# google-deepmind/mujoco_warp

Hardware: NVIDIA H100
Metric: env-steps/sec (whole box) on humanoid.xml at nworld=8192 per GPU (higher is better)
Workload: dtype f32

## Files before the change

### mujoco_warp_b200/_src/io.py

```python

from __future__ import annotations

import weakref

import numpy as np
import torch

from . import _lib
from . import constants as C
from . import mjcf
from . import types

_FLOAT_FIELDS = [
  "qpos0", "qpos_spring", "body_pos", "body_quat", "body_ipos", "body_iquat", "body_mass", "body_subtreemass",
  "body_inertia", "body_invweight0", "body_gravcomp", "jnt_pos", "jnt_axis", "jnt_stiffness", "jnt_range", "jnt_margin", "jnt_solref",
  "jnt_solimp", "jnt_actfrcrange", "dof_armature", "dof_damping", "dof_invweight0", "dof_frictionloss", "dof_solref",
  "dof_solimp", "geom_size", "geom_aabb", "geom_rbound", "geom_pos", "geom_quat", "geom_friction", "geom_margin",
  "geom_gap", "geom_solmix", "geom_solref", "geom_solimp", "actuator_gear", "actuator_gainprm", "actuator_biasprm",
  "actuator_ctrlrange", "actuator_forcerange", "cam_pos", "cam_quat", "cam_poscom0", "cam_pos0", "cam_mat0",
  "light_pos", "light_dir", "light_poscom0", "light_pos0", "light_dir0", "site_pos", "site_quat",
]
_INT_FIELDS = [
  "body_parentid", "body_rootid", "body_weldid", "body_mocapid", "body_jntnum", "body_jntadr", "body_dofnum", "body_dofadr",
  "jnt_type", "jnt_qposadr", "jnt_dofadr", "jnt_bodyid", "jnt_actfrclimited", "jnt_actgravcomp",
  "dof_bodyid", "dof_jntid", "dof_parentid", "M_rownnz", "M_rowadr", "M_colind", "tree_dofadr", "tree_dofnum",
  "geom_type", "geom_condim", "geom_bodyid", "geom_priority",
  "actuator_trnid", "actuator_gaintype", "actuator_biastype", "actuator_ctrllimited", "actuator_forcelimited",
  "cam_mode", "cam_bodyid", "cam_targetbodyid", "light_mode", "light_bodyid", "light_targetbodyid", "site_bodyid",
]
_TENDON_FLOATS = (("tendon_range", 2), ("tendon_margin", 1), ("tendon_stiffness", 1), ("tendon_damping", 1), ("tendon_frictionloss", 1), ("tendon_lengthspring", 2),
                  ("tendon_length0", 1), ("tendon_invweight0", 1), ("tendon_solref_lim", 2), ("tendon_solimp_lim", 5), ("tendon_solref_fri", 2), ("tendon_solimp_fri", 5), ("tendon_actfrcrange", 2))
_BATCHABLE_EXTRA = ("eq_solref", "eq_solimp", "eq_data", "pair_friction", "pair_solref", "pair_solreffriction", "pair_solimp", "pair_margin", "pair_gap",
                    "actuator_dynprm", "actuator_actrange", "geom_rgba", "mat_rgba", "actuator_acc0") + tuple(n for n, _ in _TENDON_FLOATS)
_SIZES = ["nq", "nv", "nu", "na", "nbody", "njnt", "ngeom", "nsite", "ncam", "nlight", "ntree", "nkey", "nmocap", "neq", "ntendon", "nflex"]

_SUPPORTED_PAIRS = {
  (C.GEOM_PLANE, C.GEOM_SPHERE), (C.GEOM_PLANE, C.GEOM_CAPSULE), (C.GEOM_SPHERE, C.GEOM_SPHERE),
  (C.GEOM_SPHERE, C.GEOM_CAPSULE), (C.GEOM_CAPSULE, C.GEOM_CAPSULE),
  (C.GEOM_PLANE, C.GEOM_ELLIPSOID), (C.GEOM_PLANE, C.GEOM_CYLINDER), (C.GEOM_PLANE, C.GEOM_BOX),
  (C.GEOM_SPHERE, C.GEOM_CYLINDER), (C.GEOM_SPHERE, C.GEOM_BOX), (C.GEOM_CAPSULE, C.GEOM_BOX),
  (C.GEOM_PLANE, C.GEOM_MESH),
}
_CONVEX_PAIRS = {
  (C.GEOM_SPHERE, C.GEOM_ELLIPSOID), (C.GEOM_CAPSULE, C.GEOM_ELLIPSOID), (C.GEOM_CAPSULE, C.GEOM_CYLINDER), (C.GEOM_ELLIPSOID, C.GEOM_ELLIPSOID),
  (C.GEOM_ELLIPSOID, C.GEOM_CYLINDER), (C.GEOM_ELLIPSOID, C.GEOM_BOX), (C.GEOM_CYLINDER, C.GEOM_CYLINDER), (C.GEOM_CYLINDER, C.GEOM_BOX),
  (C.GEOM_SPHERE, C.GEOM_MESH), (C.GEOM_CAPSULE, C.GEOM_MESH), (C.GEOM_ELLIPSOID, C.GEOM_MESH), (C.GEOM_CYLINDER, C.GEOM_MESH),
  (C.GEOM_BOX, C.GEOM_MESH), (C.GEOM_MESH, C.GEOM_MESH),
}


def _require_cuda():
  if not torch.cuda.is_available():
    raise RuntimeError("mujoco_warp_b200 runs its step path on a CUDA (sm_90a) device only; no CPU fallback exists")
  return torch.device("cuda", torch.cuda.current_device())


def is_sparse(mjm) -> bool:
  jac = getattr(mjm.opt, "jacobian", C.JAC_AUTO)
  if jac == C.JAC_AUTO:
    return mjm.nv > 32
  return jac == C.JAC_SPARSE


def _get_padded_sizes(nv: int, njmax: int, sparse: bool, tile_size: int = 16, augment_cholesky: bool = False):

  def round_up(x, m):
    return ((x + m - 1) // m) * m

  njmax_padded = round_up(njmax, tile_size)
  nv_padded = round_up(nv + int(augment_cholesky), tile_size) if (sparse or nv > 32) else round_up(nv, 4)
  return njmax_padded, nv_padded


def _default_size(base: float) -> int:
  valid = (2 + (np.arange(19) % 2)) * (2 ** (np.arange(19) // 2 + 3))
  return int(base) if base > valid[-1] else int(valid[np.searchsorted(valid, base)])


def _default_nconmax(mjm) -> int:
  return _default_size(45)


def _default_njmax(mjm) -> int:
  return _default_size(53)


def _np(mjm, name):
  return np.asarray(getattr(mjm, name))


def derive_tables(mjm) -> dict:
  nbody, nv, ngeom, njnt, nu = mjm.nbody, mjm.nv, mjm.ngeom, mjm.njnt, mjm.nu
  parent = _np(mjm, "body_parentid")
  t = {}
  depth = np.zeros(nbody, dtype=np.int32)
  for b in range(1, nbody):
    depth[b] = depth[parent[b]] + 1
  nlevel = int(depth.max()) + 1
  order = np.argsort(depth, kind="stable").astype(np.int32)
  t["level_body"] = order
  t["level_adr"] = np.searchsorted(depth[order], np.arange(nlevel + 1)).astype(np.int32)
  t["nlevel"] = nlevel
  t["body_tree"] = [order[t["level_adr"][l] : t["level_adr"][l + 1]] for l in range(nlevel)]
  children = [[] for _ in range(nbody)]
  for b in range(1, nbody):
    children[parent[b]].append(b)
  t["body_childadr"] = np.concatenate([[0], np.cumsum([len(c) for c in children])]).astype(np.int32)
  t["body_childid"] = np.array([c for cs in children for c in cs] + ([0] if nbody == 1 else []), dtype=np.int32)
  rownnz, rowadr, colind = _np(mjm, "M_rownnz"), _np(mjm, "M_rowadr"), _np(mjm, "M_colind")
  nC = int(rownnz.sum())
  entry_row = np.zeros(nC, dtype=np.int32)
  gather = [[] for _ in range(nv)]
  for i in range(nv):
    for k in range(rownnz[i]):
      e = rowadr[i] + k
      j = colind[e]
      entry_row[e] = i
      gather[i].append((j, e))
      if j != i:
        gather[j].append((i, e))
  t["nC"] = nC
  t["M_entry_row"] = entry_row
  t["mulm_rowadr"] = np.concatenate([[0], np.cumsum([len(g) for g in gather])]).astype(np.int32)
  t["mulm_col"] = np.array([c for g in gather for c, _ in sorted(g)], dtype=np.int32)
  t["mulm_madr"] = np.array([e for g in gather for _, e in sorted(g)], dtype=np.int32)
  tadr, tnum = _np(mjm, "tree_dofadr"), _np(mjm, "tree_dofnum")
  off, qadr = 0, []
  for n in tnum:
    qadr.append(off)
    off += int(n) * int(n)
  t["tree_qLDadr"] = np.array(qadr if qadr else [0], dtype=np.int32)
  t["qld_total"] = off
  t["maxtree"] = int(tnum.max()) if len(tnum) else 0
  dpar = _np(mjm, "dof_parentid")
  depth = np.zeros(max(nv, 1), dtype=np.int64)
  for i in range(nv):
    depth[i] = 1 + (depth[dpar[i]] if dpar[i] >= 0 else 0)
  t["max_dof_chain"] = int(depth.max()) if nv else 0
  blk = np.zeros(max(nv, 1), dtype=np.int32)
  for a, n, q in zip(tadr, tnum, qadr):
    blk[a : a + n] = q
  t["qLD_block_adr"] = blk
  anc = np.zeros((nbody, nv), dtype=np.int32)
  dofnum, dofadr, dparent = _np(mjm, "body_dofnum"), _np(mjm, "body_dofadr"), _np(mjm, "dof_parentid")
  for bodyid in range(nbody):
    b = bodyid
    while b > 0 and dofnum[b] == 0:
      b = parent[b]
    if dofnum[b] == 0:
      continue
    d = dofadr[b] + dofnum[b] - 1
    while d >= 0:
      anc[bodyid, d] = 1
      d = dparent[d]
  t["body_isdofancestor"] = anc
  filterparent = not (mjm.opt.disableflags & C.DSBL_FILTERPARENT)
  g1, g2 = np.triu_indices(ngeom, k=1)
  gb = _np(mjm, "geom_bodyid")
  weld = _np(mjm, "body_weldid")
  b1, b2 = gb[g1], gb[g2]
  w1, w2 = weld[b1], weld[b2]
  wp1, wp2 = weld[parent[w1]], weld[parent[w2]]
  ct, ca = _np(mjm, "geom_contype"), _np(mjm, "geom_conaffinity")
  mask = ((ct[g1] & ca[g2]) | (ct[g2] & ca[g1])).astype(bool)
  self_col = w1 == w2
  parent_child = filterparent & (w1 != 0) & (w2 != 0) & ((w1 == wp2) | (w2 == wp1))
  excl_sig = np.asarray(getattr(mjm, "exclude_signature", np.zeros(0, dtype=np.int64)))
  exclude = np.isin((b1.astype(np.int64) << 16) + b2, excl_sig)
  pairid = -np.ones(len(g1), dtype=np.int32)
  pairid[~(mask & ~self_col & ~parent_child & ~exclude)] = -2
  for i in range(int(getattr(mjm, "npair", 0))):
    a, b = sorted((int(mjm.pair_geom1[i]), int(mjm.pair_geom2[i])))
    pairid[(a * (2 * ngeom - a - 3)) // 2 + b - 1] = i
  include = pairid > -2
  t["nxn_geom_pair"] = np.stack((g1, g2), axis=1).astype(np.int32)
  t["nxn_pairid"] = np.stack((pairid, -np.ones(len(g1), dtype=np.int32)), axis=1).astype(np.int32)
  t["nxn_geom_pair_filtered"] = t["nxn_geom_pair"][include]
  t["nxn_pairid_filtered"] = t["nxn_pairid"][include]
  gt = _np(mjm, "geom_type")

  def trid(i, j):
    i, j = (j, i) if j < i else (i, j)
    return (i * (2 * C.NGEOMTYPES - i - 1)) // 2 + j

  t["has_convex_pair"] = 0
  nboxbox = nconvex = 0
  counts = np.zeros(C.NGEOMTYPES * (C.NGEOMTYPES + 1) // 2, dtype=int)
  for a, b in t["nxn_geom_pair_filtered"]:
    counts[trid(gt[a], gt[b])] += 1
    key = (min(gt[a], gt[b]), max(gt[a], gt[b]))
    if key == (C.GEOM_BOX, C.GEOM_BOX):
      if not (int(mjm.opt.disableflags) & C.DSBL_NATIVECCD):
        t["has_convex_pair"] = 1
        nboxbox += 1
        nconvex += 1
    elif key in _CONVEX_PAIRS:
      t["has_convex_pair"] = 1
      nconvex += 1
    elif key not in _SUPPORTED_PAIRS:
      raise NotImplementedError(f"collision between geom types {key} is not implemented in this version (supported: {sorted(_SUPPORTED_PAIRS | _CONVEX_PAIRS)})")
  t["geom_pair_type_count"] = tuple(int(c) for c in counts)
  t["epa_iterations"] = 16 if nboxbox == nconvex else int(getattr(mjm.opt, "ccd_iterations", 35))
  if nboxbox:
    for a, b in t["nxn_geom_pair_filtered"]:
      if gt[a] == C.GEOM_BOX and gt[b] == C.GEOM_BOX and (float(mjm.geom_margin[a]) != 0.0 or float(mjm.geom_margin[b]) != 0.0):
        raise NotImplementedError("box-box geom pair has non-zero margin with NATIVECCD enabled. Set margin to 0 or disable NATIVECCD.")
    for i in range(int(getattr(mjm, "npair", 0))):
      if gt[mjm.pair_geom1[i]] == C.GEOM_BOX and gt[mjm.pair_geom2[i]] == C.GEOM_BOX and float(mjm.pair_margin[i]) != 0.0:
        raise NotImplementedError("box-box contact pair has non-zero margin with NATIVECCD enabled. Set margin to 0 or disable NATIVECCD.")
  jt = _np(mjm, "jnt_type")
  lim = np.asarray(_np(mjm, "jnt_limited")).astype(bool)
  t["jnt_limited_slide_hinge_adr"] = np.nonzero(lim & ((jt == C.JNT_SLIDE) | (jt == C.JNT_HINGE)))[0].astype(np.int32)
  t["jnt_limited_ball_adr"] = np.nonzero(lim & (jt == C.JNT_BALL))[0].astype(np.int32)
  t["dof_fricloss_adr"] = np.nonzero(_np(mjm, "dof_frictionloss") > 0)[0].astype(np.int32)
  trnid = _np(mjm, "actuator_trnid").reshape(nu, 2)
  jdof = _np(mjm, "jnt_dofadr")
  nnz_of = {C.JNT_FREE: 6, C.JNT_BALL: 3, C.JNT_SLIDE: 1, C.JNT_HINGE: 1}
  rn, ra, ci = [], [], []
  for a in range(nu):
    trn = int(_np(mjm, "actuator_trntype")[a])
    if trn == C.TRN_TENDON:
      t_ = int(trnid[a, 0])
      adr_, n = int(_np(mjm, "ten_J_rowadr")[t_]), int(_np(mjm, "ten_J_rownnz")[t_])
      ra.append(len(ci)); rn.append(n)
      ci.extend(int(x) for x in _np(mjm, "ten_J_colind")[adr_ : adr_ + n])
      continue
    if trn != C.TRN_JOINT:
      raise NotImplementedError("only joint and tendon transmissions are implemented")
    jtype = int(jt[trnid[a, 0]])
    if jtype == C.JNT_BALL:
      raise NotImplementedError("ball-joint actuator transmission is not implemented")
    n = nnz_of[jtype]
    ra.append(len(ci))
    rn.append(n)
    ci.extend(range(jdof[trnid[a, 0]], jdof[trnid[a, 0]] + n))
  t["moment_rownnz0"] = np.array(rn if rn else [0], dtype=np.int32)
  t["moment_rowadr0"] = np.array(ra if ra else [0], dtype=np.int32)
  t["moment_colind0"] = np.array(ci if ci else [0], dtype=np.int32)
  t["nJmom"] = len(ci)
  rev = [[] for _ in range(nv)]
  for a in range(nu):
    for k in range(rn[a]):
      rev[ci[ra[a] + k]].append((a, ra[a] + k))
  t["dofact_adr"] = np.concatenate([[0], np.cumsum([len(r) for r in rev])]).astype(np.int32)
  t["dofact_act"] = np.array([a for r in rev for a, _ in r] or [0], dtype=np.int32)
  t["dofact_mom"] = np.array([i for r in rev for _, i in r] or [0], dtype=np.int32)
  nmaxcondim = int(_np(mjm, "geom_condim").max()) if ngeom else 1
  if getattr(mjm, "npair", 0):
    nmaxcondim = max(nmaxcondim, int(np.asarray(mjm.pair_dim).max()))
  t["nmaxcondim"] = nmaxcondim
  t["nmaxpyramid"] = max(1, 2 * (nmaxcondim - 1))
  return t


_COLLISION_SENSORS = (C.SENS_GEOMDIST, C.SENS_GEOMNORMAL, C.SENS_GEOMFROMTO)


def _sensor_collision_tables(mjm, t) -> dict:
  nsensor, ngeom = int(getattr(mjm, "nsensor", 0)), int(mjm.ngeom)
  stype = np.asarray(mjm.sensor_type).reshape(-1) if nsensor else np.zeros(0, dtype=int)
  sensors = np.nonzero(np.isin(stype, _COLLISION_SENSORS))[0]
  gt, gadr, gnum = _np(mjm, "geom_type"), _np(mjm, "body_geomadr"), _np(mjm, "body_geomnum")

  def geoms(objtype, objid):
    return range(int(gadr[objid]), int(gadr[objid] + gnum[objid])) if objtype == C.OBJ_BODY else range(int(objid), int(objid) + 1)

  nativeccd = not (int(mjm.opt.disableflags) & C.DSBL_NATIVECCD)
  is_ccd = lambda key: key in _CONVEX_PAIRS or (key == (C.GEOM_BOX, C.GEOM_BOX) and nativeccd)
  nccd = 0
  first = {}
  pairs, start_adr, flip, adr = [], [], [], []
  for s in sensors:
    adr.append(len(start_adr))
    for g1 in geoms(int(mjm.sensor_objtype[s]), int(mjm.sensor_objid[s])):
      for g2 in geoms(int(mjm.sensor_reftype[s]), int(mjm.sensor_refid[s])):
        a, b = min(g1, g2), max(g1, g2)
        idx = (a * (2 * ngeom - a - 3)) // 2 + b - 1
        if idx not in first:
          key = (min(gt[a], gt[b]), max(gt[a], gt[b]))
          if a == b or not (key in _SUPPORTED_PAIRS or key in _CONVEX_PAIRS or key == (C.GEOM_BOX, C.GEOM_BOX)):
            names = ("plane", "hfield", "sphere", "capsule", "ellipsoid", "cylinder", "box", "mesh", "sdf")
            raise NotImplementedError(f"collision sensor {s}: no collider for the geom types {names[key[0]]} and {names[key[1]]} (geoms {a} and {b})")
          first[idx] = len(pairs)
          lo, hi = (b, a) if gt[a] > gt[b] else (a, b)
          pairs.append((lo, hi, int(t["nxn_pairid"][idx, 0]) if t["nxn_pairid"][idx, 0] >= 0 else -1, nccd if is_ccd(key) else -1))
          nccd += is_ccd(key)
        start_adr.append(first[idx])
        flip.append(int(gt[g1] > gt[g2] or (gt[g1] == gt[g2] and g1 > g2)))
  adr.append(len(start_adr))
  convex = [(min(gt[a], gt[b]), max(gt[a], gt[b])) for a, b in list(t["nxn_geom_pair_filtered"]) + [p[:2] for p in pairs]]
  convex = [k for k in convex if is_ccd(k)]
  epa = 16 if all(k == (C.GEOM_BOX, C.GEOM_BOX) for k in convex) else int(getattr(mjm.opt, "ccd_iterations", 35))
  i32 = lambda x, shape: np.asarray(x, dtype=np.int32).reshape(shape)
  return dict(nsensorcollision=len(pairs), sensor_collision_start_adr=i32(start_adr, -1), sensor_collision_pair=i32(pairs, (len(pairs), 4)),
              sensor_collision_id=i32(sensors, -1), sensor_collision_adr=i32(adr, -1), sensor_collision_flip=i32(flip, -1), sensor_collision_epa_iterations=epa,
              nsensorcollision_ccd=nccd)


def _has_fluid(o) -> bool:
  return bool(np.any(np.asarray(getattr(o, "wind", 0.0)) != 0.0) or float(getattr(o, "density", 0.0)) > 0.0 or float(getattr(o, "viscosity", 0.0)) > 0.0)


def _validate(mjm):
  o = mjm.opt
  if o.integrator not in (C.INT_EULER, C.INT_RK4, C.INT_IMPLICIT, C.INT_IMPLICITFAST):
    raise NotImplementedError(f"unknown integrator {o.integrator}")
  if o.integrator == C.INT_IMPLICIT and 18 * mjm.nbody * 32 * 4 > 200 * 1024:
    raise NotImplementedError(f"implicit integrator: the velocity-derivative scratch of {mjm.nbody} bodies exceeds one block's shared memory (use implicitfast)")
  if o.cone not in (C.CONE_PYRAMIDAL, C.CONE_ELLIPTIC):
    raise NotImplementedError(f"unknown friction cone {o.cone}")
  if o.solver not in (C.SOL_NEWTON, C.SOL_CG):
    raise NotImplementedError("only the Newton and CG solvers are implemented in this version (no PGS)")
  if _has_fluid(o) and o.integrator == C.INT_IMPLICIT:
    raise NotImplementedError("fluid forces (opt.density / viscosity / wind) with the implicit integrator are not implemented (use implicitfast, Euler or RK4)")
  if int(getattr(o, "noslip_iterations", 0)) > 0:
    raise NotImplementedError("the noslip solver (opt.noslip_iterations > 0) is not implemented")
  unsupported_enable = int(o.enableflags) & (C.ENBL_OVERRIDE | C.ENBL_ENERGY | C.ENBL_FWDINV | C.ENBL_SLEEP)
  if unsupported_enable:
    names = [n for n, b in C.ENABLE_FLAGS.items() if unsupported_enable & b]
    raise NotImplementedError(f"enable flag(s) {names} are not implemented (contact override, energy, fwdinv, sleeping)")
  if getattr(mjm, "nu", 0):
    gt, bt = np.asarray(mjm.actuator_gaintype), np.asarray(mjm.actuator_biastype)
    if not np.isin(gt, (C.GAIN_FIXED, C.GAIN_AFFINE)).all():
      raise NotImplementedError(f"actuator gain type(s) {sorted(set(gt[~np.isin(gt, (C.GAIN_FIXED, C.GAIN_AFFINE))].tolist()))} are not implemented (fixed and affine are)")
    if not np.isin(bt, (C.BIAS_NONE, C.BIAS_AFFINE)).all():
      raise NotImplementedError(f"actuator bias type(s) {sorted(set(bt[~np.isin(bt, (C.BIAS_NONE, C.BIAS_AFFINE))].tolist()))} are not implemented (none and affine are)")
    dyn = np.asarray(getattr(mjm, "actuator_dyntype", np.zeros(mjm.nu)))
    if not np.isin(dyn, (C.DYN_NONE, C.DYN_INTEGRATOR, C.DYN_FILTER, C.DYN_FILTEREXACT)).all():
      raise NotImplementedError(f"actuator dynamics type(s) {sorted(set(dyn[~np.isin(dyn, (0, 1, 2, 3))].tolist()))} are not implemented (none, integrator, filter, filterexact are)")
  for n in ("dof_dampingpoly", "jnt_stiffnesspoly"):
    if hasattr(mjm, n) and np.any(np.asarray(getattr(mjm, n)) != 0):
      raise NotImplementedError(f"{n}: polynomial stiffness / damping is not implemented")
  gt_ = np.asarray(mjm.geom_type)
  if np.isin(gt_, (C.GEOM_HFIELD, C.GEOM_SDF)).any():
    raise NotImplementedError("height-field / SDF geoms are not implemented (plane, sphere, capsule, ellipsoid, cylinder, box and mesh geoms are)")
  if mjm.nv > 128:
    raise NotImplementedError("nv > 128 is not supported in this version (dense per-world Jacobian/Hessian in shared memory)")
  if getattr(mjm, "ntendon", 0):
    if not np.all(np.asarray(mjm.wrap_type) == C.WRAP_JOINT):
      raise NotImplementedError("spatial tendons (site / geom / pulley wraps) are not implemented; fixed tendons are")
    for n in ("tendon_armature", "tendon_stiffnesspoly", "tendon_dampingpoly"):
      if hasattr(mjm, n) and np.any(np.asarray(getattr(mjm, n)) != 0):
        raise NotImplementedError(f"{n} is not implemented")
  for n in ("nflex",):
    if getattr(mjm, n, 0):
      raise NotImplementedError(f"{n} > 0 is not supported in this version")
  if getattr(mjm, "neq", 0):
    et, ot = np.asarray(mjm.eq_type), np.asarray(mjm.eq_objtype)
    if not np.isin(et, (C.EQ_CONNECT, C.EQ_WELD, C.EQ_JOINT, C.EQ_TENDON)).all():
      raise NotImplementedError("only connect / weld / joint / tendon equality constraints are implemented")
    if (ot[np.isin(et, (C.EQ_CONNECT, C.EQ_WELD))] != C.OBJ_BODY).any():
      raise NotImplementedError("site-based connect / weld equality constraints are not implemented")
  if int(np.asarray(mjm.tree_dofnum).max(initial=0)) > 64:
    raise NotImplementedError("kinematic trees with more than 64 dofs are not supported (dense per-tree Cholesky)")


def _ptr_tensor(x: torch.Tensor) -> torch.Tensor:
  assert x.is_contiguous()
  if x.numel() == 0:
    return torch.zeros(1, dtype=x.dtype, device=x.device)
  return x


def put_model(mjm, batch_sizes=None) -> types.Model:
  batch_sizes = dict(batch_sizes or {})
  for name, size in batch_sizes.items():
    if name not in _FLOAT_FIELDS and name not in _BATCHABLE_EXTRA:
      raise ValueError(f"Model field {name!r} is not a batched array field.")
    if int(size) < 1:
      raise ValueError(f"batch_sizes[{name!r}] must be positive, got {size}.")
  dev = _require_cuda()
  L = _lib.lib()
  _validate(mjm)
  t = derive_tables(mjm)
  sparse = is_sparse(mjm)
  m = types.Model()
  for n in _SIZES:
    setattr(m, n, int(getattr(mjm, n, 0)))
  m.nC = m.nM = t["nC"]
  m.nJmom = t["nJmom"]
  m.nmaxcondim, m.nmaxpyramid = t["nmaxcondim"], t["nmaxpyramid"]
  m.is_sparse = sparse
  m.nv_pad = _get_padded_sizes(m.nv, 0, False)[1]
  m.qLD_block_total = t["qld_total"]
  m.geom_pair_type_count = t["geom_pair_type_count"]
  m.nbranch = int((t["body_childadr"][1:] - t["body_childadr"][:-1] == 0)[1:].sum()) if m.nbody > 1 else 0

  o = mjm.opt
  tol = max(float(o.tolerance), 1e-6)
  f32 = lambda x: torch.tensor(np.asarray(x, dtype=np.float32).reshape(1, *np.shape(x)), device=dev)
  m.opt = types.Option(
    timestep=f32(o.timestep), tolerance=f32(tol), ls_tolerance=f32(o.ls_tolerance), gravity=f32(np.asarray(o.gravity)),
    integrator=int(o.integrator), cone=int(o.cone), solver=int(o.solver), iterations=int(o.iterations), ls_iterations=int(o.ls_iterations),
    disableflags=int(o.disableflags), enableflags=int(o.enableflags), impratio_invsqrt=f32(1.0 / np.sqrt(o.impratio)),
    broadphase=types.BroadphaseType(int(getattr(o, "broadphase", 0))), broadphase_filter=int(getattr(o, "broadphase_filter", C.BF_PLANE | C.BF_SPHERE | C.BF_OBB)),
    graph_conditional=False, run_collision_detection=True, warn_overflow=False,
    density=f32(float(getattr(o, "density", 0.0))), viscosity=f32(float(getattr(o, "viscosity", 0.0))),
    wind=f32(np.asarray(getattr(o, "wind", np.zeros(3)), dtype=np.float64).reshape(3)),
  )
  if len(t["nxn_geom_pair_filtered"]) >= 250_000:
    raise NotImplementedError("models with >= 250k candidate geom pairs are not supported in this version")
  m.stat = types.Statistic(meaninertia=f32(mjm.stat.meaninertia))

  keep = []

  def dev_f(arr, batched=True, name=None):
    a = np.ascontiguousarray(np.asarray(arr, dtype=np.float32))
    x = torch.from_numpy(a).to(dev)
    if not batched:
      return x
    nb = int(batch_sizes.get(name, 1)) if name else 1
    return x.unsqueeze(0).repeat(nb, *([1] * x.dim())).contiguous()

  def dev_i(arr):
    a = np.ascontiguousarray(np.asarray(arr).astype(np.int32))
    return torch.from_numpy(a).to(dev)

  for n in _FLOAT_FIELDS:
    setattr(m, n, dev_f(getattr(mjm, n), name=n))
  for n in _INT_FIELDS:
    setattr(m, n, dev_i(getattr(mjm, n)))
  nu_ = int(mjm.nu)
  m.actuator_dyntype = dev_i(getattr(mjm, "actuator_dyntype", np.zeros(nu_)))
  m.actuator_actadr = dev_i(getattr(mjm, "actuator_actadr", -np.ones(nu_)))
  m.actuator_actnum = dev_i(getattr(mjm, "actuator_actnum", np.zeros(nu_)))
  m.actuator_actlimited = dev_i(np.asarray(getattr(mjm, "actuator_actlimited", np.zeros(nu_))).astype(np.int32))
  m.actuator_actearly = dev_i(np.asarray(getattr(mjm, "actuator_actearly", np.zeros(nu_))).astype(np.int32))
  m.actuator_dynprm = dev_f(np.asarray(getattr(mjm, "actuator_dynprm", np.zeros((nu_, 10)))).reshape(nu_, 10), name="actuator_dynprm")
  m.actuator_acc0 = dev_f(np.asarray(getattr(mjm, "actuator_acc0", np.zeros(nu_))).reshape(nu_), name="actuator_acc0")
  m.actuator_actrange = dev_f(np.asarray(getattr(mjm, "actuator_actrange", np.zeros((nu_, 2)))).reshape(nu_, 2), name="actuator_actrange")
  nt = int(getattr(mjm, "ntendon", 0))
  m.ntendon, m.nJten, m.nwrap = nt, (int(getattr(mjm, "nJten", 0)) if nt else 0), (int(getattr(mjm, "nwrap", 0)) if nt else 0)
  m.actuator_trntype = dev_i(getattr(mjm, "actuator_trntype", np.zeros(nu_)))
  for n in ("ten_J_rownnz", "ten_J_rowadr", "ten_J_colind", "tendon_adr", "tendon_num", "wrap_objid"):
    setattr(m, n, dev_i(getattr(mjm, n) if nt else np.zeros(0)))
  m.tendon_limited = dev_i(np.asarray(mjm.tendon_limited).astype(np.int32) if nt else np.zeros(0))
  m.tendon_actfrclimited = dev_i(np.asarray(getattr(mjm, "tendon_actfrclimited", np.zeros(nt))).astype(np.int32) if nt else np.zeros(0))
  m.wrap_prm = dev_f(mjm.wrap_prm if nt else np.zeros(0), batched=False)
  tenJ0 = np.zeros(m.nJten)
  for t_ in range(nt):
    for k in range(int(mjm.tendon_adr[t_]), int(mjm.tendon_adr[t_]) + int(mjm.tendon_num[t_])):
      dof = int(mjm.jnt_dofadr[int(mjm.wrap_objid[k])])
      row = np.asarray(mjm.ten_J_colind)[int(mjm.ten_J_rowadr[t_]) : int(mjm.ten_J_rowadr[t_]) + int(mjm.ten_J_rownnz[t_])]
      tenJ0[int(mjm.ten_J_rowadr[t_]) + int(np.nonzero(row == dof)[0][0])] = float(mjm.wrap_prm[k])
  m.ten_J0 = dev_f(tenJ0, batched=False)
  for n, k in _TENDON_FLOATS:
    setattr(m, n, dev_f(np.asarray(getattr(mjm, n)).reshape((nt, k) if k > 1 else (nt,)) if nt else np.zeros((0, k) if k > 1 else 0), name=n))
  m.ntenfric = int((np.asarray(mjm.tendon_frictionloss) > 0).sum()) if nt else 0
  m.jnt_limited = dev_i(np.asarray(mjm.jnt_limited).astype(np.int32))
  m.body_tree = tuple(dev_i(x) for x in t["body_tree"])
  for n in ("body_childadr", "body_childid", "level_adr", "level_body", "M_entry_row", "mulm_rowadr", "mulm_col", "mulm_madr", "tree_qLDadr",
            "qLD_block_adr", "jnt_limited_slide_hinge_adr", "jnt_limited_ball_adr", "dof_fricloss_adr", "moment_rownnz0", "moment_rowadr0", "moment_colind0",
            "dofact_adr", "dofact_act", "dofact_mom",
            "nxn_geom_pair", "nxn_pairid", "nxn_geom_pair_filtered", "nxn_pairid_filtered"):
    setattr(m, n, dev_i(t[n]))
  m.M_hinit_i = m.M_entry_row
  m.D_rowadr, m.D_colind, m.mapM2D = m.mulm_rowadr[:-1], m.mulm_col, m.mulm_madr
  m.D_rownnz = dev_i(np.diff(t["mulm_rowadr"]))
  m.D_diag = dev_i(np.array([list(t["mulm_col"][t["mulm_rowadr"][i] : t["mulm_rowadr"][i + 1]]).index(i) for i in range(m.nv)], dtype=np.int32))
  m.nD = int(t["mulm_rowadr"][-1])
  neq = int(getattr(mjm, "neq", 0))
  m.neq = neq
  nsensor = int(getattr(mjm, "nsensor", 0))
  unsupported = [str(x) for x in np.asarray(getattr(mjm, "sensor_unsupported", []), dtype=object).reshape(-1)]
  if unsupported:
    raise NotImplementedError(f"sensor types not implemented in this version: {sorted(set(unsupported))}")
  m.nsensor, m.nsensordata = nsensor, int(getattr(mjm, "nsensordata", 0)) if nsensor else 0
  for n in ("sensor_type", "sensor_datatype", "sensor_needstage", "sensor_objtype", "sensor_objid", "sensor_dim", "sensor_adr"):
    setattr(m, n, dev_i(getattr(mjm, n) if nsensor else np.zeros(0)))
  m.sensor_reftype = dev_i(getattr(mjm, "sensor_reftype", np.zeros(nsensor)) if nsensor else np.zeros(0))
  m.sensor_refid = dev_i(getattr(mjm, "sensor_refid", -np.ones(nsensor)) if nsensor else np.zeros(0))
  m.sensor_cutoff = dev_f(np.asarray(mjm.sensor_cutoff) if nsensor else np.zeros(0), batched=False)
  nsite = int(getattr(mjm, "nsite", 0))
  m.site_type = dev_i(getattr(mjm, "site_type", np.full(nsite, C.GEOM_SPHERE)))
  m.site_size = dev_f(getattr(mjm, "site_size", np.full((nsite, 3), 0.005)), batched=False)
  stype = np.asarray(mjm.sensor_type) if nsensor else np.zeros(0, dtype=int)
  m.sensor_subtree_vel = bool(np.isin(stype, (C.SENS_SUBTREELINVEL, C.SENS_SUBTREEANGMOM)).any())
  m.sensor_rne_postconstraint = bool(np.isin(stype, (C.SENS_ACCELEROMETER, C.SENS_FORCE, C.SENS_TORQUE, C.SENS_FRAMELINACC, C.SENS_FRAMEANGACC)).any())
  sc = _sensor_collision_tables(mjm, t)
  m.nsensorcollision, m.sensor_collision_epa_iterations, m.nsensorcollision_ccd = (sc.pop(k) for k in ("nsensorcollision", "sensor_collision_epa_iterations", "nsensorcollision_ccd"))
  for n, x in sc.items():
    setattr(m, n, dev_i(x))
  m.eq_type = dev_i(mjm.eq_type if neq else np.zeros(0))
  m.eq_obj1id = dev_i(mjm.eq_obj1id if neq else np.zeros(0))
  m.eq_obj2id = dev_i(mjm.eq_obj2id if neq else np.zeros(0))
  m.eq_objtype = dev_i(mjm.eq_objtype if neq else np.zeros(0))
  m.eq_solref = dev_f(np.asarray(mjm.eq_solref).reshape(neq, 2) if neq else np.zeros((0, 2)), name="eq_solref")
  m.eq_solimp = dev_f(np.asarray(mjm.eq_solimp).reshape(neq, 5) if neq else np.zeros((0, 5)), name="eq_solimp")
  m.eq_data = dev_f(np.asarray(mjm.eq_data).reshape(neq, 11) if neq else np.zeros((0, 11)), name="eq_data")
  npair = int(getattr(mjm, "npair", 0))
  m.npair = npair
  m.pair_dim = dev_i(mjm.pair_dim if npair else np.zeros(0))
  m.pair_geom1 = dev_i(mjm.pair_geom1 if npair else np.zeros(0))
  m.pair_geom2 = dev_i(mjm.pair_geom2 if npair else np.zeros(0))
  for n, k in (("pair_friction", 5), ("pair_solref", 2), ("pair_solreffriction", 2), ("pair_solimp", 5)):
    setattr(m, n, dev_f(np.asarray(getattr(mjm, n)).reshape(npair, k) if npair else np.zeros((0, k)), name=n))
  for n in ("pair_margin", "pair_gap"):
    setattr(m, n, dev_f(np.asarray(getattr(mjm, n)) if npair else np.zeros(0), name=n))
  nmesh = int(getattr(mjm, "nmesh", 0))
  m.nmesh = nmesh
  if nmesh and (int(getattr(mjm, "npolygonmax", 0)) > 32 or int(getattr(mjm, "nmeshdegmax", 0)) > 16):
    raise NotImplementedError(f"mesh hull with {mjm.npolygonmax} vertices in one polygon / {mjm.nmeshdegmax} polygons at one vertex: the mesh multi-contact buffers hold 32 / 16")
  m.geom_dataid = dev_i(getattr(mjm, "geom_dataid", -np.ones(m.ngeom)))
  for n in ("mesh_vertadr", "mesh_vertnum", "mesh_graphadr", "mesh_graph", "mesh_polynum", "mesh_polyadr", "mesh_polyvertadr", "mesh_polyvertnum",
            "mesh_polyvert", "mesh_polymapadr", "mesh_polymapnum", "mesh_polymap"):
    setattr(m, n, dev_i(getattr(mjm, n) if nmesh else np.zeros(0)))
  m.mesh_vert = dev_f(np.asarray(mjm.mesh_vert).reshape(-1, 3) if nmesh else np.zeros((0, 3)), batched=False)
  m.mesh_polynormal = dev_f(np.asarray(mjm.mesh_polynormal).reshape(-1, 3) if nmesh else np.zeros((0, 3)), batched=False)
  ng = m.ngeom
  m.geom_group = dev_i(getattr(mjm, "geom_group", np.zeros(ng)))
  m.geom_matid = dev_i(getattr(mjm, "geom_matid", -np.ones(ng)))
  m.geom_rgba = dev_f(np.asarray(getattr(mjm, "geom_rgba", np.tile([0.5, 0.5, 0.5, 1.0], (ng, 1)))).reshape(ng, 4), name="geom_rgba")
  m.nmat = int(getattr(mjm, "nmat", 0))
  m.mat_rgba = dev_f(np.asarray(mjm.mat_rgba).reshape(m.nmat, 4) if m.nmat else np.zeros((0, 4)), name="mat_rgba")
  m.mesh_faceadr = dev_i(getattr(mjm, "mesh_faceadr", np.zeros(nmesh)) if nmesh else np.zeros(0))
  m.mesh_face = dev_i(np.asarray(getattr(mjm, "mesh_face", np.zeros((0, 3)))).reshape(-1, 3) if nmesh else np.zeros((0, 3)))
  m.nmeshface = int(m.mesh_face.shape[0])
  m.has_fluid = _has_fluid(o)
  geom_fluid = np.asarray(getattr(mjm, "geom_fluid", np.zeros((ng, 12))), dtype=np.float64).reshape(ng, 12)
  m.geom_fluid = dev_f(geom_fluid, batched=False)
  ellipsoid = np.zeros(m.nbody, dtype=bool)
  ellipsoid[np.asarray(mjm.geom_bodyid)[geom_fluid[:, 0] > 0]] = True
  box = ~ellipsoid & (np.asarray(mjm.body_mass) > 0.0)
  box[0] = False
  m.body_fluid_ellipsoid = torch.from_numpy(ellipsoid).to(dev)
  m.body_fluid_ellipsoid_adr = dev_i(np.nonzero(ellipsoid)[0])
  m.body_fluid_box_adr = dev_i(np.nonzero(box)[0])
  m.body_fluid = dev_i(np.where(ellipsoid, 1, np.where(box, 2, 0)))
  m.body_geomadr = dev_i(mjm.body_geomadr)
  m.body_geomnum = dev_i(mjm.body_geomnum)
  m.M_mulm_rowadr, m.M_mulm_col, m.M_mulm_madr = m.mulm_rowadr, m.mulm_col, m.mulm_madr
  anc_pad = np.zeros((m.nbody, m.nv_pad), dtype=np.int32)
  anc_pad[:, : m.nv] = t["body_isdofancestor"]
  m.body_isdofancestor = dev_i(anc_pad).reshape(m.nbody, m.nv_pad)
  m._isdofancestor_nv = dev_i(t["body_isdofancestor"])
  m._mjm = mjm
  m._tables = t

  h = L.mjb_model_create()
  m._handle = h
  ints = dict(
    nq=m.nq, nv=m.nv, nu=m.nu, nbody=m.nbody, njnt=m.njnt, ngeom=m.ngeom, nsite=m.nsite, ncam=m.ncam, nlight=m.nlight, nC=m.nC, ntree=m.ntree,
    nJmom=m.nJmom, nlevel=t["nlevel"], nxn_npair=len(t["nxn_geom_pair_filtered"]), nlimit=len(t["jnt_limited_slide_hinge_adr"]),
    nfricdof=len(t["dof_fricloss_adr"]), nmaxpyramid=m.nmaxpyramid, integrator=m.opt.integrator, cone=m.opt.cone, solver=m.opt.solver,
    iterations=m.opt.iterations, ls_iterations=m.opt.ls_iterations, disableflags=m.opt.disableflags, enableflags=m.opt.enableflags,
    broadphase=int(m.opt.broadphase), broadphase_filter=m.opt.broadphase_filter, qld_total=t["qld_total"], maxtree=t["maxtree"],
    has_multicontact_geom=int(np.isin(_np(mjm, "geom_type"), (C.GEOM_ELLIPSOID, C.GEOM_CYLINDER, C.GEOM_BOX, C.GEOM_MESH)).any()), nmesh=nmesh, na=m.na, ntendon=m.ntendon, nJten=m.nJten, ntenfric=m.ntenfric, nwrap=m.nwrap,
    nmocap=int(getattr(mjm, "nmocap", 0)), npair=npair, has_convex_pair=t["has_convex_pair"], ccd_iterations=int(getattr(o, "ccd_iterations", 35)), epa_iterations=t["epa_iterations"], nsensor=m.nsensor, nsensordata=m.nsensordata, nmat=m.nmat, nmeshface=m.nmeshface, sensor_subtree_vel=int(m.sensor_subtree_vel), sensor_rne_postconstraint=int(m.sensor_rne_postconstraint), neq=neq, nlimit_ball=len(t["jnt_limited_ball_adr"]), has_fluid=int(m.has_fluid), has_gravcomp=int((np.asarray(mjm.body_gravcomp) != 0).any() or (np.asarray(mjm.jnt_stiffness)[np.isin(np.asarray(mjm.jnt_type), (C.JNT_FREE, C.JNT_BALL))] != 0).any()),
  )
  for k, v in ints.items():
    _lib.check(L.mjb_model_set_int(h, k.encode(), int(v)))
  for k, v in (("nsensorcollision", m.nsensorcollision), ("nsensorcollision_sensor", len(m.sensor_collision_id)), ("sensor_collision_epa_iterations", m.sensor_collision_epa_iterations),
               ("nsensorcollision_ccd", m.nsensorcollision_ccd)):
    _lib.check(L.mjb_model_set_int(h, k.encode(), int(v)))
  g = np.asarray(o.gravity, dtype=np.float64)
  floats = dict(timestep=o.timestep, tolerance=tol, ls_tolerance=o.ls_tolerance, impratio_invsqrt=1.0 / np.sqrt(o.impratio),
                meaninertia=mjm.stat.meaninertia, gravity_x=g[0], gravity_y=g[1], gravity_z=g[2], ccd_tolerance=float(getattr(o, "ccd_tolerance", 1e-6)))
  wind = np.asarray(getattr(o, "wind", np.zeros(3)), dtype=np.float64).reshape(3)
  floats.update(density=float(getattr(o, "density", 0.0)), viscosity=float(getattr(o, "viscosity", 0.0)), wind_x=wind[0], wind_y=wind[1], wind_z=wind[2])
  for k, v in floats.items():
    _lib.check(L.mjb_model_set_float(h, k.encode(), float(v)))
  dev_names = {
    "jnt_limited_adr": m.jnt_limited_slide_hinge_adr, "nxn_geom_pair": m.nxn_geom_pair_filtered, "nxn_pairid": m.nxn_pairid_filtered,
    "body_isdofancestor": m._isdofancestor_nv, "meaninertia": m.stat.meaninertia,
  }
  for n in (_FLOAT_FIELDS + _INT_FIELDS + ["body_childadr", "body_childid", "level_adr", "level_body", "M_entry_row", "mulm_rowadr", "mulm_col",
                                         "mulm_madr", "tree_qLDadr", "dof_fricloss_adr", "moment_rownnz0", "moment_rowadr0", "moment_colind0",
                                         "dofact_adr", "dofact_act", "dofact_mom", "eq_type", "eq_obj1id", "eq_obj2id", "eq_solref", "eq_solimp", "eq_data",
                                         "jnt_limited_ball_adr", "pair_dim", "pair_friction", "pair_solref", "pair_solreffriction", "pair_solimp",
                                         "pair_margin", "pair_gap", "sensor_type", "sensor_datatype", "sensor_needstage", "sensor_objtype", "sensor_objid", "sensor_reftype", "sensor_refid",
                                         "sensor_dim", "sensor_adr", "sensor_cutoff", "site_type", "site_size", "geom_dataid", "mesh_vertadr", "mesh_vertnum", "mesh_graphadr", "mesh_graph",
                                         "mesh_polynum", "mesh_polyadr", "mesh_polyvertadr", "mesh_polyvertnum", "mesh_polyvert", "mesh_polymapadr", "mesh_polymapnum",
                                         "mesh_polymap", "mesh_vert", "mesh_polynormal", "actuator_dyntype", "actuator_actadr", "actuator_actnum",
                                         "actuator_actlimited", "actuator_actearly", "actuator_dynprm", "actuator_actrange", "actuator_trntype",
                                         "ten_J_rownnz", "ten_J_rowadr", "ten_J_colind", "tendon_adr", "tendon_num", "wrap_objid", "tendon_limited", "tendon_actfrclimited", "wrap_prm", "ten_J0",
                                         "geom_group", "geom_matid", "geom_rgba", "mat_rgba", "mesh_faceadr", "mesh_face",
                                         "geom_fluid", "body_fluid", "body_geomadr", "body_geomnum", "sensor_collision_start_adr", "sensor_collision_pair",
                                         "sensor_collision_id", "sensor_collision_adr", "sensor_collision_flip", "actuator_acc0"]
                                        + [n for n, _ in _TENDON_FLOATS]):
    dev_names.setdefault(n, getattr(m, n))
  for n, x in dev_names.items():
    x = _ptr_tensor(x)
    keep.append(x)
    nb = int(x.shape[0]) if (n in _FLOAT_FIELDS or n in _BATCHABLE_EXTRA) and x.dim() >= 1 and x.numel() > 0 else 1
    _lib.check(L.mjb_model_set_array_batched(h, n.encode(), x.data_ptr(), nb, int(x.numel() // max(nb, 1))))
  _lib.check(L.mjb_model_finalize(h))
  m._keep = keep
  weakref.finalize(m, L.mjb_model_destroy, h)
  _install_model_rebind(m, L, set(dev_names) - {"jnt_limited_adr", "nxn_geom_pair", "nxn_pairid", "body_isdofancestor", "meaninertia"}, set(ints))
  return m


_OPT_FLOATS = {"timestep": "timestep", "tolerance": "tolerance", "ls_tolerance": "ls_tolerance", "impratio_invsqrt": "impratio_invsqrt", "ccd_tolerance": "ccd_tolerance",
               "density": "density", "viscosity": "viscosity"}
_OPT_INTS = ("integrator", "cone", "solver", "iterations", "ls_iterations", "disableflags", "enableflags", "broadphase", "broadphase_filter", "ccd_iterations")


def _check_like(name, new, old):
  if not isinstance(new, torch.Tensor):
    raise TypeError(f"{name}: expected a torch.Tensor like the bound one ({tuple(old.shape)}, {old.dtype}), got {type(new).__name__}; use .copy_() to write values")
  if new.shape != old.shape or new.dtype != old.dtype or new.device != old.device:
    raise ValueError(f"{name}: replacement must match the bound tensor: shape {tuple(old.shape)} {old.dtype} on {old.device}, got {tuple(new.shape)} {new.dtype} on {new.device}")
  return new.contiguous()


def _install_model_rebind(m: types.Model, L, arrays, ints):
  h = m._handle

  def model_hook(name, value):
    if name in arrays and name in m.__dict__:
      old = m.__dict__[name]
      batchable = name in _FLOAT_FIELDS or name in _BATCHABLE_EXTRA
      if batchable and isinstance(value, torch.Tensor) and value.dim() == old.dim() and value.shape[1:] == old.shape[1:] and value.shape[0] >= 1:
        if value.dtype != old.dtype or value.device != old.device:
          raise ValueError(f"Model.{name}: replacement must be {old.dtype} on {old.device}")
        value = value.contiguous()
      else:
        value = _check_like("Model." + name, value, old)
      x = _ptr_tensor(value)
      m._keep.append(x)
      nb = int(x.shape[0]) if batchable and x.numel() > 0 else 1
      _lib.check(L.mjb_model_set_array_batched(h, name.encode(), x.data_ptr(), nb, int(x.numel() // max(nb, 1))))
    elif name in ints and name in m.__dict__ and isinstance(m.__dict__[name], int):
      raise AttributeError(f"Model.{name} is a compiled size / table constant and cannot be reassigned; build a new Model with put_model")
    return value

  def opt_hook(name, value):
    if name in _OPT_FLOATS:
      v = float(value.reshape(-1)[0]) if isinstance(value, torch.Tensor) else float(value)
      if name == "tolerance":
        v = max(v, 1e-6)
      _lib.check(L.mjb_model_set_float(h, _OPT_FLOATS[name].encode(), v))
      return torch.full((1,), v, dtype=torch.float32, device=m.opt.__dict__[name].device) if not isinstance(value, torch.Tensor) else value
    if name in ("gravity", "wind"):
      g = value.reshape(-1)[:3].tolist() if isinstance(value, torch.Tensor) else [float(x) for x in value]
      for k, v in zip((f"{name}_x", f"{name}_y", f"{name}_z"), g):
        _lib.check(L.mjb_model_set_float(h, k.encode(), float(v)))
      return value if isinstance(value, torch.Tensor) else torch.tensor([g], dtype=torch.float32, device=m.opt.__dict__[name].device)
    if name in _OPT_INTS:
      if name == "integrator" and int(value) not in (C.INT_EULER, C.INT_IMPLICIT, C.INT_IMPLICITFAST, C.INT_RK4):
        raise NotImplementedError(f"integrator {value} not implemented")
      if name in ("integrator", "cone", "solver") and int(value) != int(m.opt.__dict__[name]):
        raise NotImplementedError(f"opt.{name} selects kernel instantiations and scratch sizes fixed at put_model / make_data; rebuild the Model to change it")
      _lib.check(L.mjb_model_set_int(h, name.encode(), int(value)))
    return value

  def stat_hook(name, value):
    if name == "meaninertia":
      v = float(value.reshape(-1)[0]) if isinstance(value, torch.Tensor) else float(value)
      _lib.check(L.mjb_model_set_float(h, b"meaninertia", v))
      old = m.stat.__dict__.get("meaninertia")
      if (isinstance(value, torch.Tensor) and value.numel() >= 1 and value.device.type != "cpu" and value.dtype == torch.float32
          and (not isinstance(old, torch.Tensor) or value.data_ptr() != old.data_ptr())):
        x = _ptr_tensor(value.contiguous())
        m._keep.append(x)
        _lib.check(L.mjb_model_set_array(h, b"meaninertia", x.data_ptr(), 1))
    return value

  object.__setattr__(m, "_rebind", model_hook)
  object.__setattr__(m.opt, "_rebind", opt_hook)
  object.__setattr__(m.stat, "_rebind", stat_hook)




def _data_spec(m: types.Model, nworld, naconmax, njmax, njmax_pad):
  f, i = torch.float32, torch.int32
  nb, nv, nq, nu, nj, ng = m.nbody, m.nv, m.nq, m.nu, m.njnt, m.ngeom
  return {
    "solver_niter": (i, (nworld,)), "ne": (i, (nworld,)), "nf": (i, (nworld,)), "nl": (i, (nworld,)), "nefc": (i, (nworld,)),
    "ten_length": (f, (nworld, m.ntendon)), "ten_J": (f, (nworld, m.nJten)), "ten_velocity": (f, (nworld, m.ntendon)),
    "time": (f, (nworld,)), "qpos": (f, (nworld, nq)), "qvel": (f, (nworld, nv)), "act": (f, (nworld, m.na)),
    "qacc_warmstart": (f, (nworld, nv)), "ctrl": (f, (nworld, nu)), "qfrc_applied": (f, (nworld, nv)), "xfrc_applied": (f, (nworld, nb, 6)),
    "qacc": (f, (nworld, nv)), "act_dot": (f, (nworld, m.na)), "sensordata": (f, (nworld, getattr(m, "nsensordata", 0))), "subtree_linvel": (f, (nworld, nb, 3)), "subtree_angmom": (f, (nworld, nb, 3)),
    "xpos": (f, (nworld, nb, 3)), "xquat": (f, (nworld, nb, 4)), "xmat": (f, (nworld, nb, 3, 3)), "xipos": (f, (nworld, nb, 3)),
    "ximat": (f, (nworld, nb, 3, 3)), "xanchor": (f, (nworld, nj, 3)), "xaxis": (f, (nworld, nj, 3)),
    "geom_xpos": (f, (nworld, ng, 3)), "geom_xmat": (f, (nworld, ng, 3, 3)), "site_xpos": (f, (nworld, m.nsite, 3)), "site_xmat": (f, (nworld, m.nsite, 3, 3)),
    "cam_xpos": (f, (nworld, m.ncam, 3)), "cam_xmat": (f, (nworld, m.ncam, 3, 3)), "light_xpos": (f, (nworld, m.nlight, 3)), "light_xdir": (f, (nworld, m.nlight, 3)),
    "subtree_com": (f, (nworld, nb, 3)), "cdof": (f, (nworld, nv, 6)), "cinert": (f, (nworld, nb, 10)),
    "actuator_length": (f, (nworld, nu)), "moment_rownnz": (i, (nworld, nu)), "moment_rowadr": (i, (nworld, nu)),
    "moment_colind": (i, (nworld, m.nJmom)), "actuator_moment": (f, (nworld, m.nJmom)),
    "crb": (f, (nworld, nb, 10)), "M": (f, (nworld, m.nC)), "qLD": (f, (nworld, m.qLD_block_total)), "qLDiagInv": (f, (nworld, nv)), "qLU": (f, (nworld, m.nD)),
    "actuator_velocity": (f, (nworld, nu)), "cvel": (f, (nworld, nb, 6)), "cdof_dot": (f, (nworld, nv, 6)),
    "qfrc_bias": (f, (nworld, nv)), "qfrc_spring": (f, (nworld, nv)), "qfrc_damper": (f, (nworld, nv)), "qfrc_gravcomp": (f, (nworld, nv)),
    "qfrc_fluid": (f, (nworld, nv)), "qfrc_adhesion": (f, (nworld, nv)), "qfrc_passive": (f, (nworld, nv)),
    "actuator_force": (f, (nworld, nu)), "qfrc_actuator": (f, (nworld, nv)), "qfrc_smooth": (f, (nworld, nv)), "qacc_smooth": (f, (nworld, nv)),
    "qfrc_constraint": (f, (nworld, nv)), "qfrc_inverse": (f, (nworld, nv)), "cacc": (f, (nworld, nb, 6)), "cfrc_int": (f, (nworld, nb, 6)),
    "cfrc_ext": (f, (nworld, nb, 6)), "energy": (f, (nworld, 2)),
    "nacon": (i, (1,)), "ncollision": (i, (1,)), "overflow": (i, (nworld,)),
    "eq_active": (i, (nworld, getattr(m, "neq", 0))),
    "mocap_pos": (f, (nworld, m.nmocap, 3)), "mocap_quat": (f, (nworld, m.nmocap, 4)),
  }


def _contact_spec(m, naconmax):
  f, i = torch.float32, torch.int32
  return {
    "dist": (f, (naconmax,)), "pos": (f, (naconmax, 3)), "frame": (f, (naconmax, 3, 3)), "includemargin": (f, (naconmax,)),
    "friction": (f, (naconmax, 5)), "solref": (f, (naconmax, 2)), "solreffriction": (f, (naconmax, 2)), "solimp": (f, (naconmax, 5)),
    "dim": (i, (naconmax,)), "geom": (i, (naconmax, 2)), "efc_address": (i, (naconmax, m.nmaxpyramid)), "worldid": (i, (naconmax,)),
    "type": (i, (naconmax,)), "geomcollisionid": (i, (naconmax,)),
  }


def _efc_spec(m, nworld, njmax, njmax_pad):
  f, i = torch.float32, torch.int32
  return {
    "type": (i, (nworld, njmax)), "id": (i, (nworld, njmax)), "J": (f, (nworld, njmax_pad, m.nv_pad)), "pos": (f, (nworld, njmax)),
    "margin": (f, (nworld, njmax)), "D": (f, (nworld, njmax_pad)), "vel": (f, (nworld, njmax)), "aref": (f, (nworld, njmax)),
    "frictionloss": (f, (nworld, njmax)), "force": (f, (nworld, njmax)), "state": (i, (nworld, njmax_pad)), "Ma": (f, (nworld, nv_of(m))),
    "Jqvel": (f, (nworld, njmax)),
  }


def nv_of(m):
  return m.nv


_BOUND_TOP = [
  "time", "qpos", "qvel", "ctrl", "qacc_warmstart", "qfrc_applied", "xfrc_applied", "qacc", "xpos", "xquat", "xmat", "xipos", "ximat", "xanchor",
  "xaxis", "geom_xpos", "geom_xmat", "site_xpos", "site_xmat", "cam_xpos", "cam_xmat", "light_xpos", "light_xdir", "subtree_com", "cdof", "cinert",
  "crb", "M", "qLD", "actuator_length", "actuator_moment", "actuator_velocity", "cvel", "cdof_dot", "qfrc_bias", "qfrc_spring", "qfrc_damper",
  "qfrc_gravcomp", "qfrc_passive", "actuator_force", "qfrc_actuator", "qfrc_smooth", "qacc_smooth", "qfrc_constraint", "qfrc_inverse", "cacc", "cfrc_int",
  "ne", "nf", "nl", "nefc", "nacon", "ncollision", "solver_niter", "overflow", "moment_rownnz", "moment_rowadr", "moment_colind", "eq_active", "mocap_pos", "mocap_quat", "sensordata", "subtree_linvel", "subtree_angmom", "cfrc_ext",
  "act", "act_dot", "ten_length", "ten_J", "ten_velocity", "qLU", "qfrc_fluid",
]
_BOUND_EFC = ["J", "pos", "margin", "D", "vel", "aref", "frictionloss", "force", "Ma", "type", "id", "state"]
_BOUND_CONTACT = ["dist", "pos", "frame", "includemargin", "friction", "solref", "solreffriction", "solimp", "dim", "geom", "efc_address", "worldid", "type", "geomcollisionid"]


def _alloc(spec, dev):
  out = {}
  for name, (dt, shape) in spec.items():
    out[name] = torch.zeros(shape, dtype=dt, device=dev)
  return out


def make_data(mjm, nworld: int = 1, nconmax=None, nccdmax=None, njmax=None, njmax_nnz=None, naconmax=None, naccdmax=None, nvmax=None, m: types.Model = None) -> types.Data:
  dev = _require_cuda()
  if m is None:
    m = put_model(mjm)
  L = _lib.lib()
  nconmax = _default_nconmax(mjm) if nconmax is None else int(nconmax)
  njmax = _default_njmax(mjm) if njmax is None else int(njmax)
  if nworld < 1:
    raise ValueError("nworld must be >= 1")
  if nconmax < 0 or njmax < 0:
    raise ValueError("nconmax and njmax must be >= 0")
  naconmax = nworld * nconmax if naconmax is None else int(naconmax)
  njmax_pad, nv_pad = _get_padded_sizes(m.nv, njmax, False)
  if m.is_sparse:
    if njmax_nnz is None:
      t = m._tables
      njmax_nnz = njmax * min(m.nv, 2 * int(t["max_dof_chain"]))
    njmax_nnz = int(njmax_nnz)
  else:
    njmax_nnz = 0
  d = types.Data(nworld=nworld, naconmax=naconmax, naccdmax=0, njmax=njmax, njmax_pad=njmax_pad, njmax_nnz=njmax_nnz, nvmax=m.nv, nconmax=nconmax)
  for k, v in _alloc(_data_spec(m, nworld, naconmax, njmax, njmax_pad), dev).items():
    setattr(d, k, v)
  d.contact = types.Contact(**_alloc(_contact_spec(m, max(naconmax, 1)), dev))
  d.efc = types.Constraint(**_alloc(_efc_spec(m, nworld, max(njmax, 1), max(njmax_pad, 1)), dev))
  i32 = torch.int32
  if m.is_sparse:
    d.efc.J_dense = d.efc.J
    d.efc.J = torch.zeros((nworld, 1, max(njmax_nnz, 1)), dtype=torch.float32, device=dev)
    d.efc.J_rownnz = torch.zeros((nworld, max(njmax, 1)), dtype=i32, device=dev)
    d.efc.J_rowadr = torch.zeros((nworld, max(njmax, 1)), dtype=i32, device=dev)
    d.efc.J_colind = torch.zeros((nworld, 1, max(njmax_nnz, 1)), dtype=i32, device=dev)
  else:
    d.efc.J_rownnz = torch.zeros((nworld, 0), dtype=i32, device=dev)
    d.efc.J_rowadr = torch.zeros((nworld, 0), dtype=i32, device=dev)
    d.efc.J_colind = torch.zeros((nworld, 0, 0), dtype=i32, device=dev)
  qpos0 = np.asarray(mjm.qpos0, dtype=np.float64)
  d.qpos.copy_(torch.from_numpy(np.tile(qpos0.astype(np.float32), (nworld, 1))))
  kin = mjcf.kinematics_np(mjm, qpos0) if hasattr(mjm, "names") else _host_kinematics(mjm, qpos0)
  d.geom_xpos.copy_(torch.from_numpy(np.tile(kin.geom_xpos.astype(np.float32), (nworld, 1, 1))))
  d.geom_xmat.copy_(torch.from_numpy(np.tile(kin.geom_xmat.astype(np.float32), (nworld, 1, 1, 1))))
  d.xquat[..., 0] = 1.0
  if getattr(m, "neq", 0):
    d.eq_active.copy_(torch.from_numpy(np.tile(np.asarray(mjm.eq_active0).astype(np.int32), (nworld, 1))))
  _reset_mocap(mjm, d)
  _bind(m, d, L)
  return d


def _reset_mocap(mjm, d):
  if not getattr(mjm, "nmocap", 0):
    return
  mid = np.asarray(mjm.body_mocapid)
  mb = np.nonzero(mid >= 0)[0]
  order = mb[np.argsort(mid[mb])]
  d.mocap_pos.copy_(torch.from_numpy(np.tile(np.asarray(mjm.body_pos, dtype=np.float32)[order], (d.nworld, 1, 1))))
  d.mocap_quat.copy_(torch.from_numpy(np.tile(np.asarray(mjm.body_quat, dtype=np.float32)[order], (d.nworld, 1, 1))))


def _host_kinematics(mjm, qpos):
  import mujoco

  mjd = mujoco.MjData(mjm)
  mjd.qpos[:] = qpos
  mujoco.mj_kinematics(mjm, mjd)
  from types import SimpleNamespace

  return SimpleNamespace(geom_xpos=np.array(mjd.geom_xpos), geom_xmat=np.array(mjd.geom_xmat).reshape(-1, 3, 3))


def _bind(m: types.Model, d: types.Data, L):
  h = L.mjb_data_create(d.nworld, d.nconmax, d.naconmax, d.njmax, d.njmax_pad, m.nv_pad)
  d._handle = h
  d._model = m
  d._keep = []

  def reg(cname, x):
    x = _ptr_tensor(x)
    d._keep.append(x)
    _lib.check(L.mjb_data_set_array(h, cname.encode(), x.data_ptr()))

  for n in _BOUND_TOP:
    reg(n, getattr(d, n))
  for n in _BOUND_EFC:
    reg("efc_" + n, d.efc.J_dense if (n == "J" and m.is_sparse) else getattr(d.efc, n))
  reg("efc_Jsp", d.efc.J if m.is_sparse else torch.zeros(1, dtype=torch.float32, device=d.efc.J.device))
  for n in ("J_rownnz", "J_rowadr", "J_colind"):
    reg("efc_" + n, getattr(d.efc, n))
  _lib.check(L.mjb_data_set_int(h, b"njmax_nnz", int(d.njmax_nnz)))
  for n in _BOUND_CONTACT:
    reg("contact_" + n, getattr(d.contact, n))
  _lib.check(L.mjb_data_finalize(h, m._handle))
  weakref.finalize(d, L.mjb_data_destroy, h)

  def make_hook(struct, prefix, names):
    def hook(name, value):
      if name in names and name in struct.__dict__:
        value = _check_like(f"{type(struct).__name__}.{name}", value, struct.__dict__[name])
        x = _ptr_tensor(value)
        d._keep.append(x)
        _lib.check(L.mjb_data_set_array(h, (prefix + name).encode(), x.data_ptr()))
      return value

    return hook

  object.__setattr__(d, "_rebind", make_hook(d, "", set(_BOUND_TOP)))
  object.__setattr__(d.efc, "_rebind", make_hook(d.efc, "efc_", (set(_BOUND_EFC) - {"J"}) if m.is_sparse else set(_BOUND_EFC)))
  object.__setattr__(d.contact, "_rebind", make_hook(d.contact, "contact_", set(_BOUND_CONTACT)))


def put_data(mjm, mjd, nworld: int = 1, nconmax=None, nccdmax=None, njmax=None, njmax_nnz=None, naconmax=None, naccdmax=None, nvmax=None, m: types.Model = None) -> types.Data:
  d = make_data(mjm, nworld, nconmax, nccdmax, njmax, njmax_nnz, naconmax, naccdmax, nvmax, m=m)
  for name in ("qpos", "qvel", "ctrl", "qacc_warmstart", "qfrc_applied", "xfrc_applied", "act"):
    if hasattr(mjd, name) and getattr(d, name).numel():
      src = np.asarray(getattr(mjd, name), dtype=np.float32)
      dst = getattr(d, name)
      dst.copy_(torch.from_numpy(np.broadcast_to(src, (nworld,) + src.shape).copy()).reshape(dst.shape))
  d.time.fill_(float(getattr(mjd, "time", 0.0)))
  return d


def reset_data(m: types.Model, d: types.Data):
  mjm = m._mjm
  d.qpos.copy_(torch.from_numpy(np.tile(np.asarray(mjm.qpos0, dtype=np.float32), (d.nworld, 1))))
  for n in ("qvel", "ctrl", "qacc_warmstart", "qacc", "qfrc_applied", "xfrc_applied", "time", "act", "act_dot"):
    getattr(d, n).zero_()
  for n in ("overflow", "solver_niter", "nefc", "ne", "nf", "nl", "nacon", "ncollision"):
    getattr(d, n).zero_()
  if getattr(m, "neq", 0):
    d.eq_active.copy_(torch.from_numpy(np.tile(np.asarray(mjm.eq_active0).astype(np.int32), (d.nworld, 1))))
  _reset_mocap(mjm, d)


def reset_data_keyframe(m: types.Model, d: types.Data, key):
  mjm = m._mjm
  nkey = int(mjm.nkey)
  if isinstance(key, (int, np.integer)):
    if key < 0 or key >= nkey:
      raise ValueError(f"key ({int(key)}) must be in [0, {nkey}).")
    keys = torch.full((d.nworld,), int(key), dtype=torch.int64, device=d.qpos.device)
  elif isinstance(key, torch.Tensor):
    if tuple(key.shape) != (d.nworld,):
      raise ValueError(f"key array must have shape ({d.nworld},), got {tuple(key.shape)}.")
    if key.dtype not in (torch.int32, torch.int64):
      raise ValueError(f"key array must be of integer type, got {key.dtype}.")
    keys = key.to(device=d.qpos.device, dtype=torch.int64)
  else:
    raise ValueError(f"key must be an int or a tensor, got {type(key)}.")
  valid = (keys >= 0) & (keys < nkey)
  if not bool(valid.any()):
    return
  idx = keys.clamp(0, max(nkey - 1, 0))
  dev = d.qpos.device
  f32 = lambda a: torch.from_numpy(np.ascontiguousarray(np.asarray(a, dtype=np.float32))).to(dev)
  sel = lambda new, old: torch.where(valid.reshape((-1,) + (1,) * (old.dim() - 1)), new, old)
  d.qpos.copy_(sel(f32(mjm.key_qpos)[idx], d.qpos))
  d.qvel.copy_(sel(f32(mjm.key_qvel)[idx], d.qvel))
  if m.nu:
    d.ctrl.copy_(sel(f32(mjm.key_ctrl)[idx], d.ctrl))
  d.time.copy_(sel(f32(mjm.key_time)[idx], d.time))
  if m.na:
    d.act.copy_(sel(f32(np.asarray(mjm.key_act).reshape(nkey, m.na))[idx], d.act))
  for n in ("qacc_warmstart", "qacc", "qfrc_applied", "xfrc_applied", "act_dot"):
    t = getattr(d, n)
    t.copy_(sel(torch.zeros_like(t), t))
  for n in ("overflow", "solver_niter", "nefc", "ne", "nf", "nl"):
    t = getattr(d, n)
    t.copy_(sel(torch.zeros_like(t), t))
  if getattr(m, "neq", 0):
    d.eq_active.copy_(sel(torch.from_numpy(np.asarray(mjm.eq_active0).astype(np.int32)).to(dev).expand(d.nworld, -1), d.eq_active))


_GET_FIELDS = (
  "qpos", "qvel", "ctrl", "qacc_warmstart", "qfrc_applied", "xfrc_applied", "qacc", "xpos", "xquat", "xmat", "xipos", "ximat", "xanchor", "xaxis",
  "geom_xpos", "geom_xmat", "site_xpos", "site_xmat", "cam_xpos", "cam_xmat", "light_xpos", "light_xdir", "subtree_com", "cdof", "cinert", "crb",
  "actuator_length", "actuator_velocity", "actuator_force", "cvel", "cdof_dot", "qfrc_bias", "qfrc_spring", "qfrc_damper", "qfrc_passive",
  "qfrc_actuator", "qfrc_smooth", "qacc_smooth", "qfrc_constraint", "cacc", "cfrc_int", "qLD", "actuator_moment",
)


def get_data_into(result, mjm, d: types.Data, world_id: int = 0):
  w = int(world_id)
  if not 0 <= w < d.nworld:
    raise ValueError(f"world_id {w} out of range [0, {d.nworld})")
  nacon = min(int(d.nacon.cpu()[0]), d.naconmax)
  nefc = min(int(d.nefc[w].cpu()), d.njmax)
  for name in _GET_FIELDS:
    setattr(result, name, getattr(d, name)[w].cpu().numpy().astype(np.float64))
  result.qM = d.M[w].cpu().numpy().astype(np.float64)
  result.M = result.qM
  result.time = float(d.time[w].cpu())
  result.solver_niter = int(d.solver_niter[w].cpu())
  result.ne, result.nf, result.nl, result.nefc = int(d.ne[w].cpu()), int(d.nf[w].cpu()), int(d.nl[w].cpu()), nefc
  ids = torch.nonzero(d.contact.worldid[:nacon] == w).reshape(-1)
  result.ncon = int(ids.numel())
  con = {}
  for name in ("dist", "pos", "frame", "includemargin", "friction", "solref", "solreffriction", "solimp", "dim", "geom", "efc_address"):
    con[name] = getattr(d.contact, name)[ids].cpu().numpy()
  result.contact = con
  nv = mjm.nv
  result.efc_J = (d.efc.J_dense if hasattr(d.efc, "J_dense") else d.efc.J)[w, :nefc, :nv].cpu().numpy().astype(np.float64)
  for name in ("pos", "margin", "D", "vel", "aref", "frictionloss", "force"):
    setattr(result, "efc_" + name, getattr(d.efc, name)[w, :nefc].cpu().numpy().astype(np.float64))
  for name in ("type", "id", "state"):
    setattr(result, "efc_" + name, getattr(d.efc, name)[w, :nefc].cpu().numpy())
  return result


def override_model(model, overrides):
  enum_fields = {
    "opt.broadphase": types.BroadphaseType, "opt.broadphase_filter": types.BroadphaseFilter, "opt.cone": types.ConeType,
    "opt.disableflags": types.DisableBit, "opt.enableflags": types.EnableBit, "opt.integrator": types.IntegratorType, "opt.solver": types.SolverType,
  }
  mj_enum_fields = {"opt.jacobian": {"DENSE": C.JAC_DENSE, "SPARSE": C.JAC_SPARSE, "AUTO": C.JAC_AUTO}}
  mjw_only = {"opt.broadphase", "opt.broadphase_filter", "opt.graph_conditional", "opt.contact_sensor_maxmatch"}
  mj_only = {"opt.jacobian", "vis.quality.offsamples"}
  is_device = isinstance(model, types.Model)
  if not isinstance(overrides, dict):
    parsed = {}
    for o in overrides:
      if "=" not in o:
        raise ValueError(f"Invalid override format: {o}")
      k, v = o.split("=", 1)
      parsed[k.strip()] = v.strip()
    overrides = parsed
  for key, val in overrides.items():
    if key in ("opt.ls_parallel", "opt.ls_parallel_min_step"):
      raise ValueError(f"{key.split('.')[1]} was removed in MuJoCo Warp 3.9.1.")
    if (key in mjw_only and not is_device) or (key in mj_only and is_device):
      continue
    obj, attrs = model, key.split(".")
    for i, attr in enumerate(attrs):
      if not hasattr(obj, attr):
        raise ValueError(f"Unrecognized model field: {key}")
      if i < len(attrs) - 1:
        obj = getattr(obj, attr)
        continue
      cur = getattr(obj, attr)
      if key in mj_enum_fields and isinstance(val, str):
        member = val.strip().upper()
        if member not in mj_enum_fields[key]:
          raise ValueError(f"Unrecognized enum value for {key}: {member}")
        val = mj_enum_fields[key][member]
      elif key in enum_fields and isinstance(val, str):
        acc = 0
        for member in val.split("|"):
          member = member.strip().upper()
          if member not in enum_fields[key].__members__:
            raise ValueError(f"Unrecognized enum value for {enum_fields[key].__name__}: {member}")
          acc |= int(enum_fields[key][member])
        val = acc
      elif isinstance(cur, bool) and isinstance(val, str):
        if val.upper() not in ("TRUE", "FALSE"):
          raise ValueError(f"Unrecognized value for field: {key}")
        val = val.upper() == "TRUE"
      elif isinstance(cur, torch.Tensor) and isinstance(val, str):
        floats = [float(p) for p in val.strip("[]").split()]
        val = torch.tensor(floats, dtype=cur.dtype, device=cur.device).reshape(cur.shape)
      elif isinstance(cur, np.ndarray) and isinstance(val, str):
        val = np.array([float(p) for p in val.strip("[]").split()], dtype=cur.dtype)
      elif isinstance(cur, torch.Tensor):
        val = torch.as_tensor(val, dtype=cur.dtype, device=cur.device).reshape(cur.shape)
      else:
        val = type(cur)(val)
      setattr(obj, attr, val)


def load_trajectory(npz_path: str, mjm, mjd) -> np.ndarray:
  data = np.load(npz_path)
  ctrl, times = data["ctrl"], data["times"]
  if ctrl.ndim != 2 or len(ctrl) == 0:
    raise ValueError(f"ctrl must have shape (nstep, nu) with nstep > 0, got {ctrl.shape}")
  if ctrl.shape[1] != mjm.nu:
    raise ValueError(f"ctrl shape {ctrl.shape} does not match model nu={mjm.nu}")
  if times.ndim != 1 or len(times) not in (len(ctrl), len(ctrl) + 1):
    raise ValueError(f"times shape {times.shape} must contain {len(ctrl)} or {len(ctrl) + 1} timestamps")
  if not np.all(np.isfinite(times)):
    raise ValueError("times must be finite")
  intervals = np.diff(times)
  if np.any(intervals <= 0):
    raise ValueError("times must be strictly increasing")
  if "qpos" in data and data["qpos"].shape[1] == mjm.nq:
    mjd.qpos[:] = data["qpos"][0]
  if "qvel" in data and data["qvel"].shape[1] == mjm.nv:
    mjd.qvel[:] = data["qvel"][0]
  if len(times) == len(ctrl):
    final_dt = intervals[-1] if len(intervals) else mjm.opt.timestep
    times = np.append(times, times[-1] + final_dt)
  n_steps = int(np.round((times[-1] - times[0]) / mjm.opt.timestep))
  sample_times = times[0] + (np.arange(n_steps) + 1e-7) * mjm.opt.timestep
  return ctrl[np.searchsorted(times, sample_times, side="right") - 1]
```

### mujoco_warp_b200/csrc/k_position.cu

```cuda

#include "mjb_math.cuh"
#include "mjb_team.cuh"
#include "mjb_types.cuh"

namespace {

struct PosLayout {
  int qpos, xpos, xquat, xipos, xanchor, xaxis, scom, cinert, cdof, buf, arena, gxpos, gxmat, M, total;
};

__host__ __device__ inline int pad4(int n) { return (n + 3) & ~3; }
__host__ __device__ inline PosLayout pos_layout(const ModelDev& m) {
  PosLayout L;
  int o = 0;
  auto take = [&](int n) { int r = o; o += pad4(n); return r; };
  L.xpos = take(3 * m.nbody); L.xquat = take(4 * m.nbody); L.xipos = take(3 * m.nbody);
  L.xanchor = take(3 * m.njnt); L.xaxis = take(3 * m.njnt); L.scom = take(3 * m.nbody);
  L.arena = take(pad4(m.nq) > pad4(9 * m.nbody) ? m.nq : 9 * m.nbody);
  L.qpos = L.arena;
  L.gxpos = L.xipos; L.gxmat = L.gxpos + pad4(3 * m.ngeom);
  L.buf = L.xpos; L.M = L.buf + pad4(6 * m.nv);
  if (o < L.gxmat + pad4(9 * m.ngeom)) o = L.gxmat + pad4(9 * m.ngeom);
  if (o < L.M + pad4(m.nC)) o = L.M + pad4(m.nC);
  L.cinert = take(10 * m.nbody); L.cdof = take(6 * m.nv);
  L.total = o;
  return L;
}

template <int LPW, bool BAT>
__global__ void __launch_bounds__(256)
k_position(const __grid_constant__ ModelDev mp, const __grid_constant__ DataDev d, int mask) {
  extern __shared__ __align__(16) float smem[];
  constexpr int G = 32 / LPW;
  Team<LPW> T;
  T.init(d.w0, d.wn, d.nworld);
  if (T.nvalid <= 0) return;
  MJB_WORLD_MODEL(T.w)
  const int lane = T.lane, sub = T.sub, g = T.g, nval = T.nvalid;
  const bool valid = T.valid;
  const PosLayout L = pos_layout(mp);
  float* S = smem + (size_t)(threadIdx.x >> 5) * ((size_t)L.total * G + 4);
  Stager st;
  st.init(reinterpret_cast<uint64_t*>(S + (size_t)L.total * G), lane);
  const int nb = m.nbody, nj = m.njnt, ng = m.ngeom, nv = m.nv;
#define BLK(f) (S + (size_t)L.f * G)
#define ROW(blk, n) ((blk) + (size_t)g * (n))
  float *qpos = ROW(BLK(qpos), m.nq), *xpos = ROW(BLK(xpos), 3 * nb), *xquat = ROW(BLK(xquat), 4 * nb), *xipos = ROW(BLK(xipos), 3 * nb),
        *xanchor = ROW(BLK(xanchor), 3 * nj), *xaxis = ROW(BLK(xaxis), 3 * nj), *scom = ROW(BLK(scom), 3 * nb), *cinert = ROW(BLK(cinert), 10 * nb),
        *cdof = ROW(BLK(cdof), 6 * nv);
  float *xmat = ROW(BLK(arena), 9 * nb), *ximat = ROW(BLK(arena), 9 * nb), *gxpos = ROW(BLK(gxpos), 3 * ng), *gxmat = ROW(BLK(gxmat), 9 * ng),
        *buf = ROW(BLK(buf), 6 * nv), *Ms = ROW(BLK(M), m.nC);
  float* crb = cinert;
  const size_t wg = (size_t)T.wg0;
#define GLOAD(blk, field, n) st.load(blk, d.field + wg * (size_t)(n), nval * (n))
#define GSTORE(field, blk, n) st.store(d.field + wg * (size_t)(n), blk, nval * (n))
  const size_t wb = (size_t)T.w;
  const bool kin = mask & STG_KINEMATICS, com = mask & STG_COM_POS, cam = mask & STG_CAMLIGHT, crbm = mask & STG_CRB;

  if (mask & (STG_KINEMATICS | STG_TRANSMISSION)) GLOAD(BLK(qpos), qpos, m.nq);
  if (!kin && (com || cam)) {
    GLOAD(BLK(xpos), xpos, 3 * nb); GLOAD(BLK(xquat), xquat, 4 * nb); GLOAD(BLK(xipos), xipos, 3 * nb);
    GLOAD(BLK(xanchor), xanchor, 3 * nj); GLOAD(BLK(xaxis), xaxis, 3 * nj);
  }
  if (!com && (cam || crbm)) { GLOAD(BLK(scom), subtree_com, 3 * nb); GLOAD(BLK(cinert), cinert, 10 * nb); GLOAD(BLK(cdof), cdof, 6 * nv); }
  st.load_wait();

  if (kin) {
    if (sub == 0) { xpos[0] = xpos[1] = xpos[2] = 0.f; xquat[0] = 1.f; xquat[1] = xquat[2] = xquat[3] = 0.f; }
    __syncwarp();
#pragma unroll 1
    for (int l = 1; l < m.nlevel; l++) {
#pragma unroll 1
      for (int i = m.level_adr[l] + sub; i < m.level_adr[l + 1]; i += LPW) {
        const int b = m.level_body[i], pid = m.body_parentid[b], jntadr = m.body_jntadr[b], jntnum = m.body_jntnum[b];
        if (jntnum == 1 && m.jnt_type[jntadr] == JNT_FREE) {
          const int qa = m.jnt_qposadr[jntadr];
          v3 p = ld3(qpos + qa);
          q4 q = qnormalize(ldq(qpos + qa + 3));
          st3(xpos + 3 * b, p); stq(xquat + 4 * b, q);
          st3(xanchor + 3 * jntadr, p); st3(xaxis + 3 * jntadr, ld3(m.jnt_axis + 3 * jntadr));
          continue;
        }
        q4 pq = ldq(xquat + 4 * pid);
        const int mc = m.nmocap > 0 ? m.body_mocapid[b] : -1;
        const v3 bpos = mc >= 0 ? ld3(d.mocap_pos + (wb * m.nmocap + mc) * 3) : ld3(m.body_pos + 3 * b);
        const q4 bquat = mc >= 0 ? ldq(d.mocap_quat + (wb * m.nmocap + mc) * 4) : ldq(m.body_quat + 4 * b);
        v3 pos = qrot(pq, bpos) + ld3(xpos + 3 * pid);
        q4 quat = qmul(pq, bquat);
#pragma unroll 1
        for (int j = jntadr; j < jntadr + jntnum; j++) {
          const int qa = m.jnt_qposadr[j], t = m.jnt_type[j];
          v3 jpos = ld3(m.jnt_pos + 3 * j), jax = ld3(m.jnt_axis + 3 * j);
          v3 anchor = qrot(quat, jpos) + pos, axis = qrot(quat, jax);
          if (t == JNT_BALL) {
            quat = qmul(quat, qnormalize(ldq(qpos + qa)));
            pos = anchor - qrot(quat, jpos);
          } else if (t == JNT_SLIDE) {
            pos = pos + axis * (qpos[qa] - m.qpos0[qa]);
          } else if (t == JNT_HINGE) {
            quat = qmul(quat, axis_angle_quat(jax, qpos[qa] - m.qpos0[qa]));
            pos = anchor - qrot(quat, jpos);
          }
          st3(xanchor + 3 * j, anchor); st3(xaxis + 3 * j, axis);
        }
        st3(xpos + 3 * b, pos); stq(xquat + 4 * b, qnormalize(quat));
      }
      __syncwarp();
    }
  }

  if (kin && m.ntendon > 0) {
#pragma unroll 1
    for (int t = valid ? sub : m.ntendon; t < m.ntendon; t += LPW) {
      d.ten_length[wb * m.ntendon + t] = tendon_length(m, t, qpos);
      for (int k = m.ten_J_rowadr[t]; k < m.ten_J_rowadr[t] + m.ten_J_rownnz[t]; k++) d.ten_J[wb * m.nJten + k] = m.ten_J0[k];
    }
  }

  if (mask & STG_TRANSMISSION) {
#pragma unroll 1
    for (int a = valid ? sub : m.nu; a < m.nu; a += LPW) {
      if (m.ntendon > 0 && m.actuator_trntype[a] == TRN_TENDON) {
        const int t = m.actuator_trnid[2 * a], adr = m.moment_rowadr0[a], nnz = m.moment_rownnz0[a], tadr = m.ten_J_rowadr[t];
        const float gear0 = m.actuator_gear[6 * a];
        d.actuator_length[wb * m.nu + a] = tendon_length(m, t, qpos) * gear0;
        d.moment_rownnz[wb * m.nu + a] = nnz;
        d.moment_rowadr[wb * m.nu + a] = adr;
        for (int k = 0; k < nnz; k++) {
          d.moment_colind[wb * m.nJmom + adr + k] = m.moment_colind0[adr + k];
          d.actuator_moment[wb * m.nJmom + adr + k] = m.ten_J0[tadr + k] * gear0;
        }
        continue;
      }
      const int j = m.actuator_trnid[2 * a], t = m.jnt_type[j], adr = m.moment_rowadr0[a], nnz = m.moment_rownnz0[a];
      const float* gear = m.actuator_gear + 6 * a;
      d.actuator_length[wb * m.nu + a] = (t == JNT_SLIDE || t == JNT_HINGE) ? qpos[m.jnt_qposadr[j]] * gear[0] : 0.f;
      d.moment_rownnz[wb * m.nu + a] = nnz;
      d.moment_rowadr[wb * m.nu + a] = adr;
#pragma unroll 1
      for (int k = 0; k < nnz; k++) {
        d.moment_colind[wb * m.nJmom + adr + k] = m.moment_colind0[adr + k];
        d.actuator_moment[wb * m.nJmom + adr + k] = gear[k];
      }
    }
  }

  __syncwarp();

  if (kin) {
#pragma unroll 2
    for (int b = sub; b < nb; b += LPW) {
      q4 q = ldq(xquat + 4 * b);
      quat_to_mat(q, xmat + 9 * b);
      st3(xipos + 3 * b, ld3(xpos + 3 * b) + qrot(q, ld3(m.body_ipos + 3 * b)));
    }
#pragma unroll 1
    for (int s = valid ? sub : m.nsite; s < m.nsite; s += LPW) {
      const int b = m.site_bodyid[s];
      q4 q = ldq(xquat + 4 * b);
      float mat[9];
      st3(d.site_xpos + (wb * m.nsite + s) * 3, ld3(xpos + 3 * b) + qrot(q, ld3(m.site_pos + 3 * s)));
      quat_to_mat(qmul(q, ldq(m.site_quat + 4 * s)), mat);
      for (int k = 0; k < 9; k++) d.site_xmat[(wb * m.nsite + s) * 9 + k] = mat[k];
    }
    st.store_fence();
    GSTORE(xpos, BLK(xpos), 3 * nb); GSTORE(xquat, BLK(xquat), 4 * nb); GSTORE(xmat, BLK(arena), 9 * nb); GSTORE(xipos, BLK(xipos), 3 * nb);
    GSTORE(xanchor, BLK(xanchor), 3 * nj); GSTORE(xaxis, BLK(xaxis), 3 * nj);
    st.store_commit();
    if (!com) {
      st.store_wait_read();
#pragma unroll 2
      for (int b = sub; b < nb; b += LPW) quat_to_mat(qmul(ldq(xquat + 4 * b), ldq(m.body_iquat + 4 * b)), ximat + 9 * b);
      st.store_fence();
      GSTORE(ximat, BLK(arena), 9 * nb);
      st.store_commit();
    }
  }
  __syncwarp();

  if (com) {
#pragma unroll 2
    for (int b = sub; b < nb; b += LPW) st3(scom + 3 * b, ld3(xipos + 3 * b) * m.body_mass[b]);
    __syncwarp();
#pragma unroll 1
    for (int l = m.nlevel - 2; l >= 0; l--) {
#pragma unroll 1
      for (int i = m.level_adr[l] + sub; i < m.level_adr[l + 1]; i += LPW) {
        const int b = m.level_body[i];
        v3 acc = ld3(scom + 3 * b);
        for (int c = m.body_childadr[b]; c < m.body_childadr[b + 1]; c++) acc = acc + ld3(scom + 3 * m.body_childid[c]);
        st3(scom + 3 * b, acc);
      }
      __syncwarp();
    }
#pragma unroll 2
    for (int b = sub; b < nb; b += LPW) {
      const float ms = m.body_subtreemass[b];
      if (ms != 0.f) st3(scom + 3 * b, ld3(scom + 3 * b) * (1.0f / ms));
    }
    __syncwarp();
    if (kin) st.store_wait_read();
#pragma unroll 2
    for (int b = sub; b < nb; b += LPW) {
      float* mat = ximat + 9 * b;
      quat_to_mat(qmul(ldq(xquat + 4 * b), ldq(m.body_iquat + 4 * b)), mat);
      const v3 inert = ld3(m.body_inertia + 3 * b);
      const float mass = m.body_mass[b];
      const v3 dif = ld3(xipos + 3 * b) - ld3(scom + 3 * m.body_rootid[b]);
      float* r = cinert + 10 * b;
      const float a0 = mat[0] * inert.x, a1 = mat[1] * inert.y, a2 = mat[2] * inert.z;
      const float b0 = mat[3] * inert.x, b1 = mat[4] * inert.y, b2 = mat[5] * inert.z;
      const float c0 = mat[6] * inert.x, c1 = mat[7] * inert.y, c2 = mat[8] * inert.z;
      r[0] = a0 * mat[0] + a1 * mat[1] + a2 * mat[2] + mass * (dif.y * dif.y + dif.z * dif.z);
      r[1] = b0 * mat[3] + b1 * mat[4] + b2 * mat[5] + mass * (dif.x * dif.x + dif.z * dif.z);
      r[2] = c0 * mat[6] + c1 * mat[7] + c2 * mat[8] + mass * (dif.x * dif.x + dif.y * dif.y);
      r[3] = a0 * mat[3] + a1 * mat[4] + a2 * mat[5] - mass * dif.x * dif.y;
      r[4] = a0 * mat[6] + a1 * mat[7] + a2 * mat[8] - mass * dif.x * dif.z;
      r[5] = b0 * mat[6] + b1 * mat[7] + b2 * mat[8] - mass * dif.y * dif.z;
      r[6] = mass * dif.x; r[7] = mass * dif.y; r[8] = mass * dif.z; r[9] = mass;
    }
#pragma unroll 2
    for (int j = sub; j < nj; j += LPW) {
      const int b = m.jnt_bodyid[j], t = m.jnt_type[j];
      int dof = m.jnt_dofadr[j];
      const v3 offset = ld3(scom + 3 * m.body_rootid[b]) - ld3(xanchor + 3 * j);
      if (t == JNT_FREE || t == JNT_BALL) {
        float xm[9];
        quat_to_mat(ldq(xquat + 4 * b), xm);
        if (t == JNT_FREE) {
          for (int k = 0; k < 18; k++) cdof[6 * dof + k] = 0.f;
          cdof[6 * dof + 3] = 1.f; cdof[6 * (dof + 1) + 4] = 1.f; cdof[6 * (dof + 2) + 5] = 1.f;
          dof += 3;
        }
        for (int k = 0; k < 3; k++) {
          v3 col = matcol(xm, k);
          st3(cdof + 6 * (dof + k), col); st3(cdof + 6 * (dof + k) + 3, cross(col, offset));
        }
      } else if (t == JNT_SLIDE) {
        st3(cdof + 6 * dof, mk3(0.f, 0.f, 0.f)); st3(cdof + 6 * dof + 3, ld3(xaxis + 3 * j));
      } else {
        v3 ax = ld3(xaxis + 3 * j);
        st3(cdof + 6 * dof, ax); st3(cdof + 6 * dof + 3, cross(ax, offset));
      }
    }
    st.store_fence();
    GSTORE(subtree_com, BLK(scom), 3 * nb); GSTORE(cinert, BLK(cinert), 10 * nb); GSTORE(cdof, BLK(cdof), 6 * nv);
    if (kin) GSTORE(ximat, BLK(arena), 9 * nb);
    st.store_commit();
  }
  __syncwarp();

  if (mask & STG_CAMLIGHT) {
#pragma unroll 1
    for (int c = valid ? sub : m.ncam; c < m.ncam; c += LPW) {
      const int mode = m.cam_mode[c], b = m.cam_bodyid[c], tb = m.cam_targetbodyid[c];
      const bool is_target = mode == CAM_TARGETBODY || mode == CAM_TARGETBODYCOM;
      v3 p; float mat[9];
      if (mode == CAM_TRACK) {
        for (int k = 0; k < 9; k++) mat[k] = m.cam_mat0[9 * c + k];
        p = ld3(xpos + 3 * b) + ld3(m.cam_pos0 + 3 * c);
      } else if (mode == CAM_TRACKCOM) {
        for (int k = 0; k < 9; k++) mat[k] = m.cam_mat0[9 * c + k];
        p = ld3(scom + 3 * b) + ld3(m.cam_poscom0 + 3 * c);
      } else if (is_target && tb >= 0) {
        q4 q = ldq(xquat + 4 * b);
        p = ld3(xpos + 3 * b) + qrot(q, ld3(m.cam_pos + 3 * c));
        v3 tp = mode == CAM_TARGETBODYCOM ? ld3(scom + 3 * tb) : ld3(xpos + 3 * tb);
        v3 m3 = normalize(p - tp), m1 = normalize(cross(mk3(0.f, 0.f, 1.f), m3)), m2 = normalize(cross(m3, m1));
        mat[0] = m1.x; mat[1] = m2.x; mat[2] = m3.x; mat[3] = m1.y; mat[4] = m2.y; mat[5] = m3.y; mat[6] = m1.z; mat[7] = m2.z; mat[8] = m3.z;
      } else {
        q4 q = ldq(xquat + 4 * b);
        p = ld3(xpos + 3 * b) + qrot(q, ld3(m.cam_pos + 3 * c));
        quat_to_mat(qmul(q, ldq(m.cam_quat + 4 * c)), mat);
      }
      st3(d.cam_xpos + (wb * m.ncam + c) * 3, p);
      for (int k = 0; k < 9; k++) d.cam_xmat[(wb * m.ncam + c) * 9 + k] = mat[k];
    }
#pragma unroll 1
    for (int l = valid ? sub : m.nlight; l < m.nlight; l += LPW) {
      const int mode = m.light_mode[l], b = m.light_bodyid[l], tb = m.light_targetbodyid[l];
      const bool is_target = mode == CAM_TARGETBODY || mode == CAM_TARGETBODYCOM;
      v3 p, dir;
      bool norm = true;
      q4 q = ldq(xquat + 4 * b);
      if (is_target && tb < 0) {
        p = ld3(xpos + 3 * b) + qrot(q, ld3(m.light_pos + 3 * l)); dir = qrot(q, ld3(m.light_dir + 3 * l)); norm = false;
      } else if (mode == CAM_TRACK) {
        dir = ld3(m.light_dir0 + 3 * l); p = ld3(xpos + 3 * b) + ld3(m.light_pos0 + 3 * l);
      } else if (mode == CAM_TRACKCOM) {
        dir = ld3(m.light_dir0 + 3 * l); p = ld3(scom + 3 * b) + ld3(m.light_poscom0 + 3 * l);
      } else if (is_target) {
        p = ld3(xpos + 3 * b) + qrot(q, ld3(m.light_pos + 3 * l));
        v3 tp = mode == CAM_TARGETBODYCOM ? ld3(scom + 3 * tb) : ld3(xpos + 3 * tb);
        dir = tp - p;
      } else {
        p = ld3(xpos + 3 * b) + qrot(q, ld3(m.light_pos + 3 * l)); dir = qrot(q, ld3(m.light_dir + 3 * l));
      }
      if (norm) dir = normalize(dir);
      st3(d.light_xpos + (wb * m.nlight + l) * 3, p);
      st3(d.light_xdir + (wb * m.nlight + l) * 3, dir);
    }
  }


  if (kin) {
    st.store_wait_read();
#pragma unroll 2
    for (int gi = sub; gi < ng; gi += LPW) {
      const int b = m.geom_bodyid[gi];
      if (m.body_weldid[b] == 0 && (m.nmocap == 0 || m.body_mocapid[m.body_rootid[b]] == -1)) {
        for (int k = 0; k < 3; k++) gxpos[3 * gi + k] = d.geom_xpos[(wb * ng + gi) * 3 + k];
        for (int k = 0; k < 9; k++) gxmat[9 * gi + k] = d.geom_xmat[(wb * ng + gi) * 9 + k];
      } else {
        q4 q = ldq(xquat + 4 * b);
        st3(gxpos + 3 * gi, ld3(xpos + 3 * b) + qrot(q, ld3(m.geom_pos + 3 * gi)));
        quat_to_mat(qmul(q, ldq(m.geom_quat + 4 * gi)), gxmat + 9 * gi);
      }
    }
    st.store_fence();
    GSTORE(geom_xpos, BLK(gxpos), 3 * ng); GSTORE(geom_xmat, BLK(gxmat), 9 * ng);
    st.store_commit();
  }

  if (crbm) {
    st.store_wait_read();
#pragma unroll 1
    for (int l = m.nlevel - 2; l >= 1; l--) {
#pragma unroll 1
      for (int i = m.level_adr[l] + sub; i < m.level_adr[l + 1]; i += LPW) {
        const int b = m.level_body[i];
        float acc[10];
#pragma unroll
        for (int k = 0; k < 10; k++) acc[k] = crb[10 * b + k];
#pragma unroll 1
        for (int c = m.body_childadr[b]; c < m.body_childadr[b + 1]; c++) {
          const float* cc = crb + 10 * m.body_childid[c];
#pragma unroll
          for (int k = 0; k < 10; k++) acc[k] += cc[k];
        }
#pragma unroll
        for (int k = 0; k < 10; k++) crb[10 * b + k] = acc[k];
      }
      __syncwarp();
    }
#pragma unroll 2
    for (int dd = sub; dd < nv; dd += LPW) inert_vec(crb + 10 * m.dof_bodyid[dd], cdof + 6 * dd, buf + 6 * dd);
    __syncwarp();
#pragma unroll 4
    for (int e = sub; e < m.nC; e += LPW) {
      const int i = m.M_entry_row[e], j = m.M_colind[e];
      float v = dot6(cdof + 6 * j, buf + 6 * i);
      if (i == j) v += m.dof_armature[i];
      Ms[e] = v;
    }
    st.store_fence();
    GSTORE(crb, BLK(cinert), 10 * nb); GSTORE(M, BLK(M), m.nC);
    st.store_commit();
  }
  st.store_wait_read();
#undef GLOAD
#undef GSTORE
#undef BLK
#undef ROW
}

}

static TeamKernel pos_kernel(const ModelDev& m, int lpw) {
  return m.batched ? k_position<32, true> : lpw == 8 ? k_position<8, false> : lpw == 16 ? k_position<16, false> : k_position<32, false>;
}

size_t smem_position(const ModelDev& m, const DataDev& d) { return team_shape(m, d.wn, pos_layout(m).total, pos_kernel).block_bytes; }
cudaError_t launch_position(const ModelDev& m, const DataDev& d, int mask, cudaStream_t s) { return team_launch(m, d, pos_layout(m).total, pos_kernel, mask, s); }
cudaError_t resident_worlds_position(const ModelDev& m, const DataDev& d, int* worlds) { return team_resident_worlds(m, d, pos_layout(m).total, pos_kernel, worlds); }
```

### mujoco_warp_b200/csrc/k_velocity.cu

```cuda

#include "mjb_fluid.cuh"
#include "mjb_math.cuh"
#include "mjb_team.cuh"
#include "mjb_types.cuh"

namespace {

struct VelLayout { int qvel, cdof, cinert, cvel, cdofdot, cacc, cfrc, qpas, qbias, qact, qsm, qld, x, af, total; };
__host__ __device__ inline VelLayout vel_layout(const ModelDev& m) {
  VelLayout L;
  int o = 0;
  auto pad = [](int n) { return (n + 3) & ~3; };
  auto take = [&](int n) { int r = o; o += pad(n); return r; };
  L.qpas = take(m.nv); L.qbias = take(m.nv);
  L.qsm = L.qpas; L.x = L.qbias;
  const int a0 = o;
  L.cdof = take(6 * m.nv); L.cinert = take(10 * m.nbody); L.qvel = take(m.nv);
  L.cvel = take(6 * m.nbody); L.cdofdot = take(6 * (m.nv > m.nbody ? m.nv : m.nbody)); L.cacc = take(6 * m.nbody);
  L.cfrc = L.cdofdot;
  if (pad(m.nv) + pad(m.nu) <= L.cvel - L.cinert) { L.qact = L.cinert; L.af = L.cinert + pad(m.nv); }
  else { L.qact = take(m.nv); L.af = take(m.nu); }
  L.qld = a0;
  if (o - a0 < pad(m.qld_total)) o = a0 + pad(m.qld_total);
  L.total = o;
  return L;
}

template <int LPW>
__device__ __forceinline__ void team_chol_upper(float* U, int n, float* x, bool solve, int sub) {
#pragma unroll 1
  for (int j = 0; j < n; j++) {
    const int iend = solve ? n + 1 : n;
#pragma unroll 1
    for (int i = j + sub; i < iend; i += LPW) {
      const bool rhs = i == n;
      const float* col = rhs ? x : U + i;
      const int cs = rhs ? 1 : n;
      float s0 = rhs ? x[j] : U[j * n + i], s1 = 0.f;
      int k = 0;
#pragma unroll 4
      for (; k + 1 < j; k += 2) {
        s0 -= U[k * n + j] * col[k * cs];
        s1 -= U[(k + 1) * n + j] * col[(k + 1) * cs];
      }
      if (k < j) s0 -= U[k * n + j] * col[k * cs];
      if (rhs) x[j] = s0 + s1; else U[j * n + i] = s0 + s1;
    }
    __syncwarp();
    const float piv = sqrtf(fmaxf(U[j * n + j], MJ_MINVAL)), inv = 1.0f / piv;
    __syncwarp();
#pragma unroll 1
    for (int i = j + sub; i < iend; i += LPW) {
      if (i == n) x[j] *= inv;
      else U[j * n + i] = i == j ? piv : U[j * n + i] * inv;
    }
    __syncwarp();
  }
  if (!solve) return;
#pragma unroll 1
  for (int j = n - 1; j >= 0; j--) {
    const float xj = x[j] / U[j * n + j];
    __syncwarp();
#pragma unroll 1
    for (int k = sub; k < j; k += LPW) x[k] -= U[k * n + j] * xj;
    if (sub == 0) x[j] = xj;
    __syncwarp();
  }
}

template <bool PEXT, int LPW, bool BAT>
__global__ void __launch_bounds__(256)
k_velocity(const __grid_constant__ ModelDev mp, const __grid_constant__ DataDev d, int mask) {
  constexpr bool FLUID = false;
  [[maybe_unused]] constexpr FluidDev f{};
#include "k_velocity_body.cuh"
}

template <int LPW, bool BAT>
__global__ void __launch_bounds__(256)
k_velocity_fluid(const __grid_constant__ ModelDev mp, const __grid_constant__ DataDev d, int mask, const __grid_constant__ FluidDev f) {
  constexpr bool PEXT = true, FLUID = true;
#include "k_velocity_body.cuh"
}

}

template <bool PEXT>
static TeamKernel vel_instance(int lpw, bool bat) {
  if (bat) return k_velocity<PEXT, 32, true>;
  return lpw == 8 ? k_velocity<PEXT, 8, false> : lpw == 16 ? k_velocity<PEXT, 16, false> : k_velocity<PEXT, 32, false>;
}
static TeamKernel vel_kernel(const ModelDev& m, int lpw) {
  return m.has_gravcomp || m.ntendon > 0 ? vel_instance<true>(lpw, m.batched) : vel_instance<false>(lpw, m.batched);
}
using FluidKernel = void (*)(ModelDev, DataDev, int, FluidDev);
static FluidKernel vel_kernel_fluid(const ModelDev& m, int lpw) {
  if (m.batched) return k_velocity_fluid<32, true>;
  return lpw == 8 ? k_velocity_fluid<8, false> : lpw == 16 ? k_velocity_fluid<16, false> : k_velocity_fluid<32, false>;
}

size_t smem_velocity(const ModelDev& m, const DataDev& d, const FluidDev& f) {
  const int words = vel_layout(m).total;
  return f.has_fluid ? team_shape(m, d.wn, words, vel_kernel_fluid).block_bytes : team_shape(m, d.wn, words, vel_kernel).block_bytes;
}
cudaError_t launch_velocity(const ModelDev& m, const DataDev& d, int mask, cudaStream_t s, const FluidDev& f) {
  const int words = vel_layout(m).total;
  return f.has_fluid ? team_launch(m, d, words, vel_kernel_fluid, mask, s, f) : team_launch(m, d, words, vel_kernel, mask, s);
}
cudaError_t resident_worlds_velocity(const ModelDev& m, const DataDev& d, int* worlds, const FluidDev& f) {
  const int words = vel_layout(m).total;
  return f.has_fluid ? team_resident_worlds(m, d, words, vel_kernel_fluid, worlds) : team_resident_worlds(m, d, words, vel_kernel, worlds);
}
```

### mujoco_warp_b200/csrc/k_velocity_body.cuh

```cuda
  extern __shared__ __align__(16) float smem[];
  constexpr int G = 32 / LPW;
  Team<LPW> T;
  T.init(d.w0, d.wn, d.nworld);
  if (T.nvalid <= 0) return;
  MJB_WORLD_MODEL(T.w)
  const int lane = T.lane, sub = T.sub, g = T.g, nval = T.nvalid;
  const bool valid = T.valid;
  const VelLayout L = vel_layout(mp);
  float* S = smem + (size_t)(threadIdx.x >> 5) * ((size_t)L.total * G + 4);
  Stager st;
  st.init(reinterpret_cast<uint64_t*>(S + (size_t)L.total * G), lane);
  const int nv = m.nv, nb = m.nbody, nu = m.nu;
#define FLD(f, n) (S + (size_t)L.f * G + (size_t)g * (n))
  float *qvel = FLD(qvel, nv), *cdof = FLD(cdof, 6 * nv), *cinert = FLD(cinert, 10 * nb), *cvel = FLD(cvel, 6 * nb), *cdofdot = FLD(cdofdot, 6 * nv),
        *cacc = FLD(cacc, 6 * nb), *cfrc = FLD(cfrc, 6 * nb), *q_passive = FLD(qpas, nv), *q_bias = FLD(qbias, nv), *q_act = FLD(qact, nv),
        *q_smooth = FLD(qsm, nv), *qld = FLD(qld, m.qld_total), *x = FLD(x, nv), *aforce = FLD(af, nu);
  const float* Mw = d.M + (size_t)T.w * m.nC;
#undef FLD
  const size_t wg = (size_t)T.wg0;
#define GLOAD(f, field, n) st.load(S + (size_t)L.f * G, d.field + wg * (size_t)(n), nval * (n))
#define GSTORE(field, f, n) st.store(d.field + wg * (size_t)(n), S + (size_t)L.f * G, nval * (n))
  const size_t wb = (size_t)T.w;
  const bool v_all = mask & STG_VELOCITY;

  GLOAD(qvel, qvel, nv); GLOAD(cdof, cdof, 6 * nv);
  if (v_all || (mask & STG_RNE)) GLOAD(cinert, cinert, 10 * nb);
  constexpr int MREG = 32;
  float mreg[MREG];
  const bool fac = mask & (STG_ACCELERATION | STG_FACTOR_ONLY);
#pragma unroll
  for (int k = 0; k < MREG; k++) { const int e = sub + k * LPW; mreg[k] = (fac && e < m.nC) ? Mw[e] : 0.f; }
  bool any_xfrc = false;
  if (mask & STG_ACCELERATION) {
#pragma unroll 4
    for (int i = sub; i < 6 * nb; i += LPW) any_xfrc |= d.xfrc_applied[wb * 6 * nb + i] != 0.f;
  }
  st.load_wait();

  if (mask & (STG_VELOCITY | STG_COMVEL | STG_PASSIVE | STG_RNE)) {
    if (v_all)
#pragma unroll 1
    for (int a = valid ? sub : nu; a < nu; a += LPW) {
      const int nnz = d.moment_rownnz[wb * nu + a], adr = d.moment_rowadr[wb * nu + a];
      float vel = 0.f;
      for (int k = 0; k < nnz; k++) vel += d.actuator_moment[wb * m.nJmom + adr + k] * qvel[d.moment_colind[wb * m.nJmom + adr + k]];
      d.actuator_velocity[wb * nu + a] = vel;
    }
    if (PEXT && v_all && m.ntendon > 0) {
#pragma unroll 1
      for (int t = valid ? sub : m.ntendon; t < m.ntendon; t += LPW) {
        float vel = 0.f;
        for (int k = m.ten_J_rowadr[t]; k < m.ten_J_rowadr[t] + m.ten_J_rownnz[t]; k++) vel += m.ten_J0[k] * qvel[m.ten_J_colind[k]];
        d.ten_velocity[wb * m.ntendon + t] = vel;
      }
    }
    if (v_all || (mask & STG_COMVEL)) {
    if (sub < 6) cvel[sub] = 0.f;
    __syncwarp();
#pragma unroll 1
    for (int l = 1; l < m.nlevel; l++) {
#pragma unroll 1
      for (int i = m.level_adr[l] + sub; i < m.level_adr[l + 1]; i += LPW) {
        const int b = m.level_body[i], pid = m.body_parentid[b], jntadr = m.body_jntadr[b], jntnum = m.body_jntnum[b];
        int dof = m.body_dofadr[b];
        float cv[6];
#pragma unroll
        for (int k = 0; k < 6; k++) cv[k] = cvel[6 * pid + k];
#pragma unroll 1
        for (int j = jntadr; j < jntadr + jntnum; j++) {
          const int t = m.jnt_type[j];
          if (t == JNT_FREE) {
            for (int q = 0; q < 3; q++) { const float v = qvel[dof + q]; for (int k = 0; k < 6; k++) { cv[k] += cdof[6 * (dof + q) + k] * v; cdofdot[6 * (dof + q) + k] = 0.f; } }
            for (int q = 3; q < 6; q++) motion_cross(cv, cdof + 6 * (dof + q), cdofdot + 6 * (dof + q));
            for (int q = 3; q < 6; q++) { const float v = qvel[dof + q]; for (int k = 0; k < 6; k++) cv[k] += cdof[6 * (dof + q) + k] * v; }
            dof += 6;
          } else if (t == JNT_BALL) {
            for (int q = 0; q < 3; q++) motion_cross(cv, cdof + 6 * (dof + q), cdofdot + 6 * (dof + q));
            for (int q = 0; q < 3; q++) { const float v = qvel[dof + q]; for (int k = 0; k < 6; k++) cv[k] += cdof[6 * (dof + q) + k] * v; }
            dof += 3;
          } else {
            motion_cross(cv, cdof + 6 * dof, cdofdot + 6 * dof);
            const float v = qvel[dof];
            for (int k = 0; k < 6; k++) cv[k] += cdof[6 * dof + k] * v;
            dof += 1;
          }
        }
#pragma unroll
        for (int k = 0; k < 6; k++) cvel[6 * b + k] = cv[k];
      }
      __syncwarp();
    }
    st.store_fence();
    GSTORE(cvel, cvel, 6 * nb); GSTORE(cdof_dot, cdofdot, 6 * nv);
    st.store_commit();
    } else if (mask & STG_RNE) {
      GLOAD(cvel, cvel, 6 * nb); GLOAD(cdofdot, cdof_dot, 6 * nv);
      st.load_wait();
    }

    if (v_all || (mask & STG_PASSIVE)) {
      const bool dsbl_spring = m.disableflags & DSBL_SPRING, dsbl_damper = m.disableflags & DSBL_DAMPER;
      const bool gravcomp = PEXT && m.has_gravcomp && !(m.disableflags & DSBL_GRAVITY) && !(dsbl_spring && dsbl_damper);
      [[maybe_unused]] const bool fluid = FLUID && !(dsbl_spring && dsbl_damper);
      if constexpr (FLUID) if (fluid) {
        const float* cv = (v_all || (mask & STG_COMVEL)) ? cvel : d.cvel + wb * 6 * nb;
        const float *xip = d.xipos + wb * nb * 3, *stc = d.subtree_com + wb * nb * 3;
#pragma unroll 1
        for (int b = sub; b < nb; b += LPW)
          fluid_body_wrench(m, f, b, cv + 6 * b, ld3(xip + 3 * b), d.ximat + (wb * nb + b) * 9, ld3(stc + 3 * m.body_rootid[b]), d.geom_xpos + wb * m.ngeom * 3,
                            d.geom_xmat + wb * m.ngeom * 9, cacc + 6 * b);
        __syncwarp();
      }
#pragma unroll 1
      for (int dd = sub; dd < nv; dd += LPW) {
        const int j = m.dof_jntid[dd], t = m.jnt_type[j];
        float spring = 0.f, damper = 0.f, gc = 0.f;
        if (!(dsbl_spring && dsbl_damper)) {
          const float stiffness = m.jnt_stiffness[j];
          if (stiffness != 0.f && !dsbl_spring) {
            const int qa = m.jnt_qposadr[j], k = dd - m.jnt_dofadr[j];
            if (t == JNT_SLIDE || t == JNT_HINGE) spring = -(d.qpos[wb * m.nq + qa] - m.qpos_spring[qa]) * stiffness;
            else if (!PEXT) {}
            else if (t == JNT_FREE && k < 3) spring = -stiffness * (d.qpos[wb * m.nq + qa + k] - m.qpos_spring[qa + k]);
            else {
              const int ra = t == JNT_FREE ? qa + 3 : qa, kk = t == JNT_FREE ? k - 3 : k;
              const q4 rot = qnormalize(ldq(d.qpos + wb * m.nq + ra)), ref = ldq(m.qpos_spring + ra);
              const q4 qd = qmul(mkq(ref.w, -ref.x, -ref.y, -ref.z), rot);
              const float s2 = sqrtf(qd.x * qd.x + qd.y * qd.y + qd.z * qd.z);
              if (s2 != 0.f) {
                float speed = 2.0f * atan2f(s2, qd.w);
                if (speed > 3.14159265358979f) speed -= 2.0f * 3.14159265358979f;
                spring = -stiffness * (kk == 0 ? qd.x : kk == 1 ? qd.y : qd.z) * (speed / s2);
              }
            }
          }
          const float damping = m.dof_damping[dd];
          if (damping != 0.f && !dsbl_damper) damper = -qvel[dd] * damping;
          if (PEXT && m.ntendon > 0) {
#pragma unroll 1
            for (int tn = 0; tn < m.ntendon; tn++) {
              const float ks = m.tendon_stiffness[tn], kd = m.tendon_damping[tn];
              if ((ks == 0.f || dsbl_spring) && (kd == 0.f || dsbl_damper)) continue;
              const float J = tendon_J_at(m, tn, dd);
              if (J == 0.f) continue;
              if (ks != 0.f && !dsbl_spring) {
                const float len = d.ten_length[wb * m.ntendon + tn], lo = m.tendon_lengthspring[2 * tn], hi = m.tendon_lengthspring[2 * tn + 1];
                const float x = len > hi ? len - hi : (len < lo ? len - lo : 0.f);
                spring += J * (-x * ks);
              }
              if (kd != 0.f && !dsbl_damper) {
                float vel = 0.f;
                for (int k = m.ten_J_rowadr[tn]; k < m.ten_J_rowadr[tn] + m.ten_J_rownnz[tn]; k++) vel += m.ten_J0[k] * qvel[m.ten_J_colind[k]];
                damper += J * (-vel * kd);
              }
            }
          }
        }
        if (gravcomp) {
#pragma unroll 1
          for (int b = 1; b < nb; b++) {
            const float g = m.body_gravcomp[b];
            if (g == 0.f || !m.body_isdofancestor[b * nv + dd]) continue;
            const float sc = -m.body_mass[b] * g;
            const v3 off = ld3(d.xipos + (wb * nb + b) * 3) - ld3(d.subtree_com + (wb * nb + m.body_rootid[b]) * 3);
            const v3 jp = ld3(cdof + 6 * dd + 3) + cross(ld3(cdof + 6 * dd), off);
            gc += sc * (jp.x * m.gravity_x + jp.y * m.gravity_y + jp.z * m.gravity_z);
          }
        }
        float passive = spring + damper + (m.jnt_actgravcomp[j] ? 0.f : gc);
        if constexpr (FLUID) {
          const float fl = fluid ? fluid_project(m, dd, cdof + 6 * dd, cacc, d.xipos + wb * nb * 3, d.subtree_com + wb * nb * 3) : 0.f;
          passive += fl;
          if (valid) f.qfrc_fluid[wb * nv + dd] = fl;
        }
        q_passive[dd] = passive;
        if (valid) {
          d.qfrc_spring[wb * nv + dd] = spring;
          d.qfrc_damper[wb * nv + dd] = damper;
          d.qfrc_gravcomp[wb * nv + dd] = gc;
          d.qfrc_passive[wb * nv + dd] = passive;
        }
      }
    }
    if (v_all || (mask & STG_RNE)) {
    for (int k = sub; k < 6; k += LPW) cacc[k] = k < 3 ? 0.f : ((m.disableflags & DSBL_GRAVITY) ? 0.f : -(k == 3 ? m.gravity_x : k == 4 ? m.gravity_y : m.gravity_z));
    __syncwarp();
#pragma unroll 1
    for (int l = 1; l < m.nlevel; l++) {
#pragma unroll 1
      for (int i = m.level_adr[l] + sub; i < m.level_adr[l + 1]; i += LPW) {
        const int b = m.level_body[i], pid = m.body_parentid[b];
        float a[6];
#pragma unroll
        for (int k = 0; k < 6; k++) a[k] = cacc[6 * pid + k];
#pragma unroll 1
        for (int q = 0; q < m.body_dofnum[b]; q++) {
          const int dof = m.body_dofadr[b] + q;
          const float v = qvel[dof];
#pragma unroll
          for (int k = 0; k < 6; k++) a[k] += cdofdot[6 * dof + k] * v;
        }
#pragma unroll
        for (int k = 0; k < 6; k++) cacc[6 * b + k] = a[k];
      }
      __syncwarp();
    }
    st.store_wait_read();
#pragma unroll 2
    for (int b = sub; b < nb; b += LPW) {
      float f[6] = {0.f, 0.f, 0.f, 0.f, 0.f, 0.f};
      if (b > 0) {
        float iv[6], g[6];
        inert_vec(cinert + 10 * b, cacc + 6 * b, f);
        inert_vec(cinert + 10 * b, cvel + 6 * b, iv);
        motion_cross_force(cvel + 6 * b, iv, g);
#pragma unroll
        for (int k = 0; k < 6; k++) f[k] += g[k];
      }
#pragma unroll
      for (int k = 0; k < 6; k++) cfrc[6 * b + k] = f[k];
    }
    __syncwarp();
#pragma unroll 1
    for (int l = m.nlevel - 2; l >= 0; l--) {
#pragma unroll 1
      for (int i = m.level_adr[l] + sub; i < m.level_adr[l + 1]; i += LPW) {
        const int b = m.level_body[i];
        float acc[6];
#pragma unroll
        for (int k = 0; k < 6; k++) acc[k] = cfrc[6 * b + k];
#pragma unroll 1
        for (int c = m.body_childadr[b]; c < m.body_childadr[b + 1]; c++) {
          const float* cc = cfrc + 6 * m.body_childid[c];
#pragma unroll
          for (int k = 0; k < 6; k++) acc[k] += cc[k];
        }
#pragma unroll
        for (int k = 0; k < 6; k++) cfrc[6 * b + k] = acc[k];
      }
      __syncwarp();
    }
#pragma unroll 1
    for (int dd = sub; dd < nv; dd += LPW) {
      const float v = dot6(cdof + 6 * dd, cfrc + 6 * m.dof_bodyid[dd]);
      q_bias[dd] = v;
    }
    st.store_fence();
    GSTORE(cacc, cacc, 6 * nb); GSTORE(cfrc_int, cfrc, 6 * nb); GSTORE(qfrc_bias, qbias, nv);
    st.store_commit();
    }
  } else if (mask & STG_ACCELERATION) {
    GLOAD(qpas, qfrc_passive, nv); GLOAD(qbias, qfrc_bias, nv);
    st.load_wait();
  }
  __syncwarp();

  if (mask & STG_ACTUATION) {
#pragma unroll 1
    for (int dd = sub; dd < nv; dd += LPW) q_act[dd] = 0.f;
    __syncwarp();
    const bool enabled = nu > 0 && !(m.disableflags & DSBL_ACTUATION);
#pragma unroll 1
    for (int a = sub; a < nu; a += LPW) {
      float force = 0.f;
      if (enabled) {
        float ctrl = d.ctrl[wb * nu + a];
        if (m.actuator_ctrllimited[a] && !(m.disableflags & DSBL_CLAMPCTRL)) ctrl = clampf(ctrl, m.actuator_ctrlrange[2 * a], m.actuator_ctrlrange[2 * a + 1]);
        const float length = d.actuator_length[wb * nu + a], velocity = d.actuator_velocity[wb * nu + a];
        const float *gp = m.actuator_gainprm + 10 * a, *bp = m.actuator_biasprm + 10 * a;
        float gain = 0.f, bias = 0.f;
        if (m.actuator_gaintype[a] == GAIN_FIXED) gain = gp[0];
        else if (m.actuator_gaintype[a] == GAIN_AFFINE) gain = gp[0] + gp[1] * length + gp[2] * velocity;
        if (m.actuator_biastype[a] == BIAS_AFFINE) bias = bp[0] + bp[1] * length + bp[2] * velocity;
        float ctrl_act = ctrl;
        if (m.na > 0 && m.actuator_actadr[a] >= 0) {
          const int last = m.actuator_actadr[a] + m.actuator_actnum[a] - 1, dyn = m.actuator_dyntype[a];
          const float act = d.act[wb * m.na + last];
          float act_dot = 0.f;
          if (dyn == DYN_INTEGRATOR) act_dot = ctrl;
          else if (dyn == DYN_FILTER || dyn == DYN_FILTEREXACT) act_dot = (ctrl - act) / fmaxf(m.actuator_dynprm[10 * a], MJ_MINVAL);
          if (valid) d.act_dot[wb * m.na + last] = act_dot;
          ctrl_act = m.actuator_actearly[a] ? next_act(m, a, act, act_dot, 1.0f, m.actuator_actlimited[a] != 0) : act;
        }
        force = gain * ctrl_act + bias;
        if (m.actuator_forcelimited[a]) force = clampf(force, m.actuator_forcerange[2 * a], m.actuator_forcerange[2 * a + 1]);
      } else if (m.na > 0 && m.actuator_actadr[a] >= 0 && valid) {
        d.act_dot[wb * m.na + m.actuator_actadr[a] + m.actuator_actnum[a] - 1] = 0.f;
      }
      if (valid) d.actuator_force[wb * nu + a] = force;
      aforce[a] = force;
    }
    __syncwarp();
    if (PEXT && enabled && m.ntendon > 0) {
#pragma unroll 1
      for (int t = sub; t < m.ntendon; t += LPW) {
        if (!m.tendon_actfrclimited[t]) continue;
        float total = 0.f;
        for (int b = 0; b < nu; b++) if (m.actuator_trntype[b] == TRN_TENDON && m.actuator_trnid[2 * b] == t) total += aforce[b];
        const float lo = m.tendon_actfrcrange[2 * t], hi = m.tendon_actfrcrange[2 * t + 1];
        const float sc = total < lo ? lo / total : (total > hi ? hi / total : 1.0f);
        if (sc == 1.0f) continue;
        for (int b = 0; b < nu; b++)
          if (m.actuator_trntype[b] == TRN_TENDON && m.actuator_trnid[2 * b] == t) { aforce[b] *= sc; if (valid) d.actuator_force[wb * nu + b] = aforce[b]; }
      }
      __syncwarp();
    }
    if (enabled) {
#pragma unroll 1
      for (int dd = sub; dd < nv; dd += LPW) {
        float q = 0.f;
        for (int k = m.dofact_adr[dd]; k < m.dofact_adr[dd + 1]; k++) q += d.actuator_moment[wb * m.nJmom + m.dofact_mom[k]] * aforce[m.dofact_act[k]];
        const int j = m.dof_jntid[dd];
        if (!(m.disableflags & DSBL_GRAVITY) && m.jnt_actgravcomp[j]) q += d.qfrc_gravcomp[wb * nv + dd];
        if (m.jnt_actfrclimited[j]) q = clampf(q, m.jnt_actfrcrange[2 * j], m.jnt_actfrcrange[2 * j + 1]);
        q_act[dd] = q;
      }
    }
    st.store_fence();
    GSTORE(qfrc_actuator, qact, nv);
    st.store_commit();
  } else if (mask & STG_ACCELERATION) {
    GLOAD(qact, qfrc_actuator, nv);
    st.load_wait();
  }
  __syncwarp();

  if (mask & (STG_ACCELERATION | STG_FACTOR_ONLY)) {
    if (mask & STG_ACCELERATION) {
#pragma unroll 1
      for (int dd = sub; dd < nv; dd += LPW) q_smooth[dd] = q_passive[dd] - q_bias[dd] + q_act[dd] + d.qfrc_applied[wb * nv + dd];
      if (team_any<LPW>(any_xfrc, g)) {
#pragma unroll 1
        for (int dd = sub; dd < nv; dd += LPW) {
          const float* cd = cdof + 6 * dd;
          const int db = m.dof_bodyid[dd];
          float acc = 0.f;
          for (int b = db; b < nb; b++) {
            const float* ft = d.xfrc_applied + (wb * nb + b) * 6;
            if (ft[0] == 0.f && ft[1] == 0.f && ft[2] == 0.f && ft[3] == 0.f && ft[4] == 0.f && ft[5] == 0.f) continue;
            int p = b;
            while (p != 0 && p != db) p = m.body_parentid[p];
            if (p == 0) continue;
            const v3 off = ld3(d.xipos + (wb * nb + b) * 3) - ld3(d.subtree_com + (wb * nb + m.body_rootid[b]) * 3);
            const v3 cr = cross(ld3(cd), off);
            acc += cd[3] * ft[0] + cd[4] * ft[1] + cd[5] * ft[2] + cd[0] * ft[3] + cd[1] * ft[4] + cd[2] * ft[5] + dot(cr, ld3(ft));
          }
          q_smooth[dd] += acc;
        }
      }
      __syncwarp();
    }
    const bool acc = mask & STG_ACCELERATION;
    st.store_wait_read();
#pragma unroll 1
    for (int i = sub; i < m.qld_total; i += LPW) qld[i] = 0.f;
    if (acc)
#pragma unroll 1
      for (int i = sub; i < nv; i += LPW) x[i] = q_smooth[i];
    __syncwarp();
#pragma unroll 1
    for (int t = 0; t < m.ntree; t++) {
      const int start = m.tree_dofadr[t], n = m.tree_dofnum[t];
      float* U = qld + m.tree_qLDadr[t];
      const int e0 = m.M_rowadr[start], e1 = m.M_rowadr[start + n - 1] + m.M_rownnz[start + n - 1];
#pragma unroll
      for (int k = 0; k < MREG; k++) {
        const int e = sub + k * LPW;
        if (e >= e0 && e < e1) U[(m.M_colind[e] - start) * n + (m.M_entry_row[e] - start)] = mreg[k];
      }
#pragma unroll 1
      for (int e = max(e0, MREG * LPW) + ((sub - max(e0, MREG * LPW)) % LPW + LPW) % LPW; e < e1; e += LPW)
        U[(m.M_colind[e] - start) * n + (m.M_entry_row[e] - start)] = Mw[e];
      __syncwarp();
      team_chol_upper<LPW>(U, n, x + start, acc, sub);
    }
    st.store_fence();
    if (acc) { GSTORE(qfrc_smooth, qsm, nv); GSTORE(qacc_smooth, x, nv); }
    GSTORE(qLD, qld, m.qld_total);
    st.store_commit();
  }
  st.store_wait_read();
#undef GLOAD
#undef GSTORE
```

### mujoco_warp_b200/csrc/mjb_team.cuh

```cuda
#pragma once
#include <algorithm>
#include <climits>
#include <cstdint>
#include <cuda_runtime.h>

#include "mjb_launch.cuh"
#include "mjb_math.cuh"
#include "mjb_types.cuh"

template <int LPW>
__device__ __forceinline__ float team_sum(float v) {
#pragma unroll
  for (int o = LPW / 2; o > 0; o >>= 1) v += __shfl_xor_sync(FULL_MASK, v, o);
  return v;
}
template <int LPW>
__device__ __forceinline__ int team_sum_i(int v) {
#pragma unroll
  for (int o = LPW / 2; o > 0; o >>= 1) v += __shfl_xor_sync(FULL_MASK, v, o);
  return v;
}
template <int LPW>
__device__ __forceinline__ bool team_any(bool p, int g) {
  const unsigned b = __ballot_sync(FULL_MASK, p);
  return LPW == 32 ? b != 0u : ((b >> (g * LPW)) & ((1u << (LPW & 31)) - 1u)) != 0u;
}

__device__ __forceinline__ uint32_t smem_u32(const void* p) { return (uint32_t)__cvta_generic_to_shared(p); }

struct Stager {
  uint64_t* bar;
  uint32_t phase;
  int lane;
  bool pending_store;

  __device__ __forceinline__ void init(uint64_t* b, int lane_) {
    bar = b; phase = 0; lane = lane_; pending_store = false;
    if (lane == 0) {
      asm volatile("mbarrier.init.shared::cta.b64 [%0], 1;" ::"r"(smem_u32(bar)) : "memory");
      asm volatile("fence.mbarrier_init.release.cluster;" ::: "memory");
    }
    __syncwarp();
  }
  static __device__ __forceinline__ bool bulk_ok(const void* g, const void* s, int nfloats) {
    return (((uintptr_t)g | (uintptr_t)smem_u32(s)) & 15u) == 0 && (nfloats & 3) == 0 && nfloats > 0;
  }
  __device__ __forceinline__ void load(float* s, const float* g, int n) {
    if (bulk_ok(g, s, n)) {
      if (lane == 0) {
        const uint32_t bytes = (uint32_t)n * 4u;
        asm volatile("mbarrier.expect_tx.relaxed.cta.shared::cta.b64 [%0], %1;" ::"r"(smem_u32(bar)), "r"(bytes) : "memory");
        asm volatile("cp.async.bulk.shared::cluster.global.mbarrier::complete_tx::bytes [%0], [%1], %2, [%3];" ::"r"(smem_u32(s)), "l"(g),
                     "r"(bytes), "r"(smem_u32(bar))
                     : "memory");
      }
    } else {
#pragma unroll 1
      for (int i = lane; i < n; i += 32) s[i] = g[i];
    }
  }
  __device__ __forceinline__ void load_wait() {
    if (lane == 0) asm volatile("mbarrier.arrive.shared::cta.b64 _, [%0];" ::"r"(smem_u32(bar)) : "memory");
    uint32_t ok = 0;
    while (!ok) {
      asm volatile("{\n .reg .pred p;\n mbarrier.try_wait.parity.shared::cta.b64 p, [%1], %2;\n selp.u32 %0, 1, 0, p;\n}" : "=r"(ok) : "r"(smem_u32(bar)), "r"(phase) : "memory");
    }
    phase ^= 1u;
    __syncwarp();
  }
  __device__ __forceinline__ void store_fence() {
    asm volatile("fence.proxy.async.shared::cta;" ::: "memory");
    __syncwarp();
  }
  __device__ __forceinline__ void store(float* g, const float* s, int n) {
    if (bulk_ok(g, s, n)) {
      if (lane == 0) {
        asm volatile("cp.async.bulk.global.shared::cta.bulk_group [%0], [%1], %2;" ::"l"(g), "r"(smem_u32(s)), "r"((uint32_t)n * 4u) : "memory");
        pending_store = true;
      }
    } else {
#pragma unroll 1
      for (int i = lane; i < n; i += 32) g[i] = s[i];
    }
  }
  __device__ __forceinline__ void store_commit() {
    if (lane == 0 && pending_store) asm volatile("cp.async.bulk.commit_group;" ::: "memory");
  }
  __device__ __forceinline__ void store_wait_read() {
    if (lane == 0 && pending_store) { asm volatile("cp.async.bulk.wait_group.read 0;" ::: "memory"); pending_store = false; }
    __syncwarp();
  }
};

using TeamKernel = void (*)(ModelDev, DataDev, int);
template <class K>
using TeamChooserOf = K (*)(const ModelDev& m, int lpw);

struct TeamShape { int lpw, wpb; size_t block_bytes; };
template <class K>
inline TeamShape team_shape(const ModelDev& m, int nworld, size_t world_words, TeamChooserOf<K> kernel_of) {
  constexpr size_t kBlockMax = 200 * 1024;
  auto bytes = [&](int lpw) { return (world_words * (size_t)(32 / lpw) + 4) * sizeof(float); };
  int lpw = 8;
  while (lpw < 32 && bytes(lpw) > kBlockMax / 2) lpw *= 2;
  int wpb = 2;
  if (m.batched && lpw < 32) {
    lpw = 32;
  } else {
    const SmLimits& sm = sm_limits();
    const long groups = (nworld + 32 / lpw - 1) / (32 / lpw);
    const int warp_regs = (kernel_regs(kernel_of(m, lpw)) * 32 + 255) & ~255;
    auto rounds = [&](int w) {
      long per_sm = (long)(sm.smem_per_sm / sm_block_bytes(bytes(lpw) * w));
      per_sm = std::min({per_sm, (long)sm.blocks, (long)(sm.warps / w)});
      if (warp_regs > 0) per_sm = std::min(per_sm, (long)(sm.regs / warp_regs / w));
      const long fit = per_sm * sm.sms, blocks = (groups + w - 1) / w;
      return fit > 0 ? (blocks + fit - 1) / fit : LONG_MAX;
    };
    for (int w : {1, 4})
      if (bytes(lpw) * w <= kBlockMax && rounds(w) < rounds(wpb)) wpb = w;
  }
  while (wpb > 1 && bytes(lpw) * wpb > kBlockMax) wpb--;
  return TeamShape{lpw, wpb, bytes(lpw) * wpb};
}

inline int team_carveout(size_t block_bytes) {
  const size_t per_sm = sm_limits().smem_per_sm, block = sm_block_bytes(block_bytes), fit = per_sm / block;
  const size_t pct = fit > 0 ? (100 * fit * block + per_sm - 1) / per_sm : 100;
  return pct < 100 ? (int)pct : (int)cudaSharedmemCarveoutMaxShared;
}

template <class K, class... A>
inline cudaError_t team_launch(const ModelDev& m, const DataDev& d, size_t world_words, TeamChooserOf<K> kernel_of, int mask, cudaStream_t s, const A&... extra) {
  const TeamShape t = team_shape(m, d.wn, world_words, kernel_of);
  const int G = 32 / t.lpw, ngroups = (d.wn + G - 1) / G, grid = (ngroups + t.wpb - 1) / t.wpb;
  return launch(kernel_of(m, t.lpw), grid, 32 * t.wpb, t.block_bytes, team_carveout(t.block_bytes), s, m, d, mask, extra...);
}

template <class K>
inline cudaError_t team_resident_worlds(const ModelDev& m, const DataDev& d, size_t world_words, TeamChooserOf<K> kernel_of, int* worlds) {
  const TeamShape t = team_shape(m, d.wn, world_words, kernel_of);
  const K kern = kernel_of(m, t.lpw);
  int blocks = 0;
  cudaError_t e = launch_configure((const void*)kern, t.block_bytes, team_carveout(t.block_bytes));
  if (e == cudaSuccess) e = cudaOccupancyMaxActiveBlocksPerMultiprocessor(&blocks, kern, 32 * t.wpb, t.block_bytes);
  *worlds = blocks * t.wpb * (32 / t.lpw);
  return e;
}

template <int LPW>
struct Team {
  static constexpr int G = 32 / LPW;
  int lane, sub, g;
  int wg0, nvalid;
  int w;
  bool valid;
  __device__ __forceinline__ void init(int w0, int wn, int nworld) {
    lane = threadIdx.x & 31; sub = lane % LPW; g = lane / LPW;
    wg0 = w0 + (blockIdx.x * (blockDim.x >> 5) + (threadIdx.x >> 5)) * G;
    const int wend = min(w0 + wn, nworld);
    nvalid = min(G, wend - wg0);
    valid = g < nvalid;
    w = wg0 + (valid ? g : nvalid - 1);
  }
};
```

### mujoco_warp_b200/csrc/mjb_types.cuh

```cuda
#pragma once
#include <cuda_runtime.h>

#define MJB_MODEL_INTS(X) \
  X(nq) X(nv) X(nu) X(nbody) X(njnt) X(ngeom) X(nsite) X(ncam) X(nlight) X(nC) X(ntree) X(nJmom) X(nlevel) \
  X(nxn_npair) X(nlimit) X(nfricdof) X(nmaxpyramid) X(integrator) X(cone) X(solver) X(iterations) \
  X(ls_iterations) X(disableflags) X(enableflags) X(broadphase) X(broadphase_filter) X(qld_total) X(maxtree) X(has_multicontact_geom) X(neq) X(nlimit_ball) X(has_gravcomp) X(nmocap) X(npair) X(has_convex_pair) X(ccd_iterations) X(epa_iterations) X(nsensor) X(nsensordata) X(sensor_subtree_vel) X(sensor_rne_postconstraint) X(nmesh) X(na) X(ntendon) X(nJten) X(ntenfric) X(nwrap) X(nmat) X(nmeshface)
#define MJB_MODEL_FLOATS(X) \
  X(timestep) X(tolerance) X(ls_tolerance) X(impratio_invsqrt) X(meaninertia) X(gravity_x) X(gravity_y) X(gravity_z) X(ccd_tolerance)
#define MJB_MODEL_IARRS(X) \
  X(body_parentid) X(body_rootid) X(body_weldid) X(body_mocapid) X(body_jntnum) X(body_jntadr) X(body_dofnum) X(body_dofadr) \
  X(body_childadr) X(body_childid) X(level_adr) X(level_body) \
  X(jnt_type) X(jnt_qposadr) X(jnt_dofadr) X(jnt_bodyid) X(jnt_actfrclimited) X(jnt_actgravcomp) X(jnt_limited_adr) \
  X(dof_bodyid) X(dof_jntid) X(dof_parentid) X(dof_fricloss_adr) X(M_rownnz) X(M_rowadr) X(M_colind) X(M_entry_row) X(mulm_rowadr) X(mulm_col) X(mulm_madr) \
  X(tree_dofadr) X(tree_dofnum) X(tree_qLDadr) \
  X(geom_type) X(geom_condim) X(geom_bodyid) X(geom_priority) \
  X(actuator_trnid) X(actuator_gaintype) X(actuator_biastype) X(actuator_ctrllimited) X(actuator_forcelimited) \
  X(actuator_dyntype) X(actuator_actadr) X(actuator_actnum) X(actuator_actlimited) X(actuator_actearly) X(actuator_trntype) \
  X(ten_J_rownnz) X(ten_J_rowadr) X(ten_J_colind) X(tendon_adr) X(tendon_num) X(wrap_objid) X(tendon_limited) X(tendon_actfrclimited) \
  X(moment_rownnz0) X(moment_rowadr0) X(moment_colind0) X(dofact_adr) X(dofact_act) X(dofact_mom) \
  X(cam_mode) X(cam_bodyid) X(cam_targetbodyid) X(light_mode) X(light_bodyid) X(light_targetbodyid) X(site_bodyid) \
  X(nxn_geom_pair) X(nxn_pairid) X(body_isdofancestor) X(eq_type) X(eq_obj1id) X(eq_obj2id) X(jnt_limited_ball_adr) X(pair_dim) \
  X(sensor_type) X(sensor_datatype) X(sensor_needstage) X(sensor_objtype) X(sensor_objid) X(sensor_reftype) X(sensor_refid) X(sensor_dim) X(sensor_adr) X(site_type) \
  X(geom_dataid) X(mesh_vertadr) X(mesh_vertnum) X(mesh_graphadr) X(mesh_graph) X(mesh_polynum) X(mesh_polyadr) X(mesh_polyvertadr) X(mesh_polyvertnum) \
  X(mesh_polyvert) X(mesh_polymapadr) X(mesh_polymapnum) X(mesh_polymap) X(geom_group) X(geom_matid) X(mesh_faceadr) X(mesh_face)
#define MJB_MODEL_FARRS(X) \
  X(qpos0) X(qpos_spring) X(body_pos) X(body_quat) X(body_ipos) X(body_iquat) X(body_mass) X(body_subtreemass) \
  X(body_inertia) X(body_invweight0) X(body_gravcomp) X(jnt_pos) X(jnt_axis) X(jnt_stiffness) X(jnt_range) X(jnt_margin) X(jnt_solref) \
  X(jnt_solimp) X(jnt_actfrcrange) X(dof_armature) X(dof_damping) X(dof_invweight0) X(dof_frictionloss) X(dof_solref) \
  X(dof_solimp) X(geom_size) X(geom_aabb) X(geom_rbound) X(geom_pos) X(geom_quat) X(geom_friction) X(geom_margin) \
  X(geom_gap) X(geom_solmix) X(geom_solref) X(geom_solimp) X(actuator_gear) X(actuator_gainprm) X(actuator_biasprm) \
  X(actuator_ctrlrange) X(actuator_forcerange) X(cam_pos) X(cam_quat) X(cam_poscom0) X(cam_pos0) X(cam_mat0) \
  X(light_pos) X(light_dir) X(light_poscom0) X(light_pos0) X(light_dir0) X(site_pos) X(site_quat) \
  X(eq_solref) X(eq_solimp) X(eq_data) X(pair_friction) X(pair_solref) X(pair_solreffriction) X(pair_solimp) X(pair_margin) X(pair_gap) \
  X(sensor_cutoff) X(site_size) X(mesh_vert) X(mesh_polynormal) X(actuator_dynprm) X(actuator_actrange) \
  X(wrap_prm) X(ten_J0) X(tendon_range) X(tendon_margin) X(tendon_stiffness) X(tendon_damping) X(tendon_frictionloss) X(tendon_lengthspring) \
  X(tendon_length0) X(tendon_invweight0) X(tendon_solref_lim) X(tendon_solimp_lim) X(tendon_solref_fri) X(tendon_solimp_fri) X(tendon_actfrcrange) \
  X(geom_rgba) X(mat_rgba)

struct ModelDev {
#define X(n) int n;
  MJB_MODEL_INTS(X)
#undef X
#define X(n) float n;
  MJB_MODEL_FLOATS(X)
#undef X
#define X(n) const int* __restrict__ n;
  MJB_MODEL_IARRS(X)
#undef X
#define X(n) const float* __restrict__ n;
  MJB_MODEL_FARRS(X)
#undef X
  int batched;
#define X(n) int nb_##n, bs_##n;
  MJB_MODEL_FARRS(X)
#undef X
};

#ifdef __CUDACC__
__device__ __forceinline__ ModelDev world_model(const ModelDev& m, int w, int nworld) {
  ModelDev r = m;
#define X(n) if (m.nb_##n > 1) r.n = m.n + (size_t)(m.nb_##n == nworld ? w : w % m.nb_##n) * (size_t)m.bs_##n;
  MJB_MODEL_FARRS(X)
#undef X
  return r;
}
#define MJB_WORLD_MODEL(w)                                         \
  ModelDev m_world_;                                               \
  if (BAT) m_world_ = world_model(mp, (w), d.nworld);              \
  const ModelDev& m = BAT ? m_world_ : mp;
#endif

#define MJB_DATA_FARRS(X) \
  X(time) X(qpos) X(qvel) X(ctrl) X(qacc_warmstart) X(qfrc_applied) X(xfrc_applied) X(qacc) \
  X(xpos) X(xquat) X(xmat) X(xipos) X(ximat) X(xanchor) X(xaxis) X(geom_xpos) X(geom_xmat) X(site_xpos) X(site_xmat) \
  X(cam_xpos) X(cam_xmat) X(light_xpos) X(light_xdir) X(subtree_com) X(cdof) X(cinert) X(crb) X(M) X(qLD) \
  X(actuator_length) X(actuator_moment) X(actuator_velocity) X(cvel) X(cdof_dot) X(qfrc_bias) X(qfrc_spring) \
  X(qfrc_damper) X(qfrc_gravcomp) X(qfrc_passive) X(actuator_force) X(qfrc_actuator) X(qfrc_smooth) X(qacc_smooth) \
  X(qfrc_constraint) X(cacc) X(cfrc_int) \
  X(efc_J) X(efc_pos) X(efc_margin) X(efc_D) X(efc_vel) X(efc_aref) X(efc_frictionloss) X(efc_force) X(efc_Ma) \
  X(contact_dist) X(contact_pos) X(contact_frame) X(contact_includemargin) X(contact_friction) X(contact_solref) \
  X(contact_solreffriction) X(contact_solimp) X(mocap_pos) X(mocap_quat) X(sensordata) X(subtree_linvel) X(subtree_angmom) X(cfrc_ext) X(efc_Jsp) X(act) X(act_dot) X(ten_length) X(ten_J) X(ten_velocity) X(qLU)
#define MJB_DATA_IARRS(X) \
  X(ne) X(nf) X(nl) X(nefc) X(nacon) X(ncollision) X(solver_niter) X(overflow) X(efc_type) X(efc_id) X(efc_state) \
  X(moment_rownnz) X(moment_rowadr) X(moment_colind) X(contact_dim) X(contact_geom) X(contact_efc_address) \
  X(contact_worldid) X(contact_type) X(contact_geomcollisionid) X(eq_active) X(efc_J_rownnz) X(efc_J_rowadr) X(efc_J_colind)

struct DataDev {
  int nworld, nconmax, naconmax, njmax, njmax_pad, nv_pad;
  int w0, wn;
  int njmax_nnz;
#define X(n) float* __restrict__ n;
  MJB_DATA_FARRS(X)
#undef X
#define X(n) int* __restrict__ n;
  MJB_DATA_IARRS(X)
#undef X
  int* world_conadr;
  int* world_ncon;
  float* imp_qacc;
};

#define MJB_FLUID_INTS(X) X(has_fluid)
#define MJB_FLUID_FLOATS(X) X(density) X(viscosity) X(wind_x) X(wind_y) X(wind_z)
#define MJB_FLUID_IARRS(X) X(body_fluid) X(body_geomadr) X(body_geomnum)
#define MJB_FLUID_FARRS(X) X(geom_fluid)
struct FluidDev {
  int has_fluid;
  float density, viscosity, wind_x, wind_y, wind_z;
  const int* __restrict__ body_fluid;
  const int* __restrict__ body_geomadr;
  const int* __restrict__ body_geomnum;
  const float* __restrict__ geom_fluid;
  float* __restrict__ qfrc_fluid;
};

#define MJB_SENSCOL_INTS(X) X(nsensorcollision) X(nsensorcollision_sensor) X(nsensorcollision_ccd) X(sensor_collision_epa_iterations)
#define MJB_SENSCOL_IARRS(X) X(sensor_collision_start_adr) X(sensor_collision_pair) X(sensor_collision_id) X(sensor_collision_adr) X(sensor_collision_flip)
struct SensorCollisionDev {
  int nsensorcollision;
  int nsensorcollision_sensor;
  int nsensorcollision_ccd;
  int sensor_collision_epa_iterations;
  const int* __restrict__ sensor_collision_start_adr;
  const int* __restrict__ sensor_collision_pair;
  const int* __restrict__ sensor_collision_id;
  const int* __restrict__ sensor_collision_adr;
  const int* __restrict__ sensor_collision_flip;
};

struct SetConstDev {
  float* __restrict__ actuator_acc0;
  int nb_actuator_acc0;
  float* __restrict__ meaninertia;
  float* __restrict__ qpos_save;
};
enum { QPOS_SAVE_LOAD0 = 0, QPOS_SAVE_LOADSPRING = 1, QPOS_LOADSPRING = 2, QPOS_RESTORE = 3 };

enum { JNT_FREE = 0, JNT_BALL = 1, JNT_SLIDE = 2, JNT_HINGE = 3 };
enum { GEOM_PLANE = 0, GEOM_HFIELD, GEOM_SPHERE, GEOM_CAPSULE, GEOM_ELLIPSOID, GEOM_CYLINDER, GEOM_BOX, GEOM_MESH };
enum { INT_EULER = 0, INT_RK4, INT_IMPLICIT, INT_IMPLICITFAST };
enum { CONE_PYRAMIDAL = 0, CONE_ELLIPTIC = 1 };
enum { SOL_CG = 1, SOL_NEWTON = 2 };
enum { EQ_CONNECT = 0, EQ_WELD = 1, EQ_JOINT = 2, EQ_TENDON = 3 };
enum { TRN_JOINT = 0, TRN_TENDON = 3 };
enum { OBJ_BODY = 1, OBJ_XBODY = 2, OBJ_GEOM = 5, OBJ_SITE = 6, OBJ_CAMERA = 7 };
enum { SENS_TOUCH = 0, SENS_ACCELEROMETER = 1, SENS_VELOCIMETER = 2, SENS_GYRO = 3, SENS_FORCE = 4, SENS_TORQUE = 5, SENS_JOINTPOS = 9, SENS_JOINTVEL = 10, SENS_TENDONPOS = 11, SENS_TENDONVEL = 12, SENS_ACTUATORPOS = 13, SENS_ACTUATORVEL = 14,
       SENS_ACTUATORFRC = 15, SENS_JOINTACTFRC = 16, SENS_BALLQUAT = 18, SENS_BALLANGVEL = 19, SENS_JOINTLIMITPOS = 20, SENS_JOINTLIMITVEL = 21, SENS_JOINTLIMITFRC = 22, SENS_FRAMEPOS = 26, SENS_FRAMEQUAT = 27, SENS_FRAMEXAXIS = 28,
       SENS_FRAMEYAXIS = 29, SENS_FRAMEZAXIS = 30, SENS_FRAMELINVEL = 31, SENS_FRAMEANGVEL = 32, SENS_FRAMELINACC = 33, SENS_FRAMEANGACC = 34, SENS_SUBTREECOM = 35, SENS_SUBTREELINVEL = 36, SENS_SUBTREEANGMOM = 37, SENS_GEOMDIST = 39, SENS_GEOMNORMAL = 40,
       SENS_GEOMFROMTO = 41, SENS_CLOCK = 45 };
enum { CNSTR_EQUALITY = 0, CNSTR_FRICTION_DOF = 1, CNSTR_FRICTION_TENDON = 2, CNSTR_LIMIT_JOINT = 3, CNSTR_LIMIT_TENDON = 4, CNSTR_CONTACT_FRICTIONLESS = 5, CNSTR_CONTACT_PYRAMIDAL = 6, CNSTR_CONTACT_ELLIPTIC = 7 };
enum { ST_SATISFIED = 0, ST_QUADRATIC = 1, ST_LINEARNEG = 2, ST_LINEARPOS = 3, ST_CONE = 4 };
enum { CAM_FIXED = 0, CAM_TRACK, CAM_TRACKCOM, CAM_TARGETBODY, CAM_TARGETBODYCOM };
enum { GAIN_FIXED = 0, GAIN_AFFINE = 1 };
enum { DYN_NONE = 0, DYN_INTEGRATOR = 1, DYN_FILTER = 2, DYN_FILTEREXACT = 3 };
enum { BIAS_NONE = 0, BIAS_AFFINE = 1 };
enum {
  DSBL_CONSTRAINT = 1 << 0, DSBL_EQUALITY = 1 << 1, DSBL_FRICTIONLOSS = 1 << 2, DSBL_LIMIT = 1 << 3, DSBL_CONTACT = 1 << 4,
  DSBL_SPRING = 1 << 5, DSBL_DAMPER = 1 << 6, DSBL_GRAVITY = 1 << 7, DSBL_CLAMPCTRL = 1 << 8, DSBL_WARMSTART = 1 << 9,
  DSBL_ACTUATION = 1 << 11, DSBL_REFSAFE = 1 << 12, DSBL_SENSOR = 1 << 13, DSBL_EULERDAMP = 1 << 15, DSBL_NATIVECCD = 1 << 17
};
enum { ENBL_INVDISCRETE = 1 << 3 };
enum { OVF_NEFC = 1 << 0, OVF_NJMAX_NNZ = 1 << 1, OVF_BROADPHASE = 1 << 2, OVF_NARROWPHASE = 1 << 3, OVF_EPA_HORIZON = 1 << 8, OVF_ITERATIONS = 1 << 9, OVF_LS_ITERATIONS = 1 << 10 };
enum { BF_PLANE = 1, BF_SPHERE = 2, BF_AABB = 4, BF_OBB = 8 };
enum { CONTACT_TYPE_CONSTRAINT = 1, CONTACT_TYPE_SENSOR = 2 };

#define MJ_MINVAL 1e-15f
#define MJ_MAXVAL 1e10f
#define MJ_MINIMP 1e-4f
#define MJ_MAXIMP 0.9999f
#define MJ_MINMU 1e-5f

enum { STG_KINEMATICS = 1, STG_COM_POS = 2, STG_CAMLIGHT = 4, STG_CRB = 8, STG_TRANSMISSION = 16 };
enum { STG_VELOCITY = 1, STG_ACTUATION = 2, STG_ACCELERATION = 4, STG_FACTOR_ONLY = 8,
       STG_COMVEL = 16, STG_PASSIVE = 32, STG_RNE = 64 };

cudaError_t launch_position(const ModelDev& m, const DataDev& d, int stage_mask, cudaStream_t s);
cudaError_t launch_collision(const ModelDev& m, const DataDev& d, cudaStream_t s);
cudaError_t launch_collision_mesh(const ModelDev& m, const DataDev& d, cudaStream_t s);
size_t smem_collision_mesh(const ModelDev& m, const DataDev& d);
cudaError_t reset_contact_counters(const DataDev& d, cudaStream_t s);
cudaError_t launch_constraint(const ModelDev& m, const DataDev& d, cudaStream_t s);
cudaError_t launch_efc_csr(const ModelDev& m, const DataDev& d, cudaStream_t s);
cudaError_t launch_velocity(const ModelDev& m, const DataDev& d, int stage_mask, cudaStream_t s, const FluidDev& f);
cudaError_t launch_solve_m(const ModelDev& m, const DataDev& d, float* x, const float* y, cudaStream_t s);
cudaError_t launch_mul_m(const ModelDev& m, const DataDev& d, float* res, const float* vec, cudaStream_t s);
cudaError_t launch_solver(const ModelDev& m, const DataDev& d, cudaStream_t s);
cudaError_t launch_integrate(const ModelDev& m, const DataDev& d, int integrator, cudaStream_t s, const FluidDev& f);
cudaError_t launch_implicit_solve(const ModelDev& m, const DataDev& d, float* qacc_out, cudaStream_t s);
size_t smem_implicit(const ModelDev& m);
cudaError_t launch_sensor(const ModelDev& m, const DataDev& d, int stages, cudaStream_t s, const SensorCollisionDev& c);
cudaError_t launch_sensor_collision(const ModelDev& m, const DataDev& d, const SensorCollisionDev& c, cudaStream_t s);
size_t smem_sensor_collision(const SensorCollisionDev& c);
cudaError_t launch_contact_force(const ModelDev& m, const DataDev& d, const int* contact_ids, int n, int to_world, float* out, cudaStream_t s);
cudaError_t launch_inverse(const ModelDev& m, const DataDev& d, float* qfrc_inverse, float* qacc_cont, bool disc, cudaStream_t s, const FluidDev& f);
cudaError_t launch_rk_stage(const ModelDev& m, const DataDev& d, float* rk, int stage, cudaStream_t s);
cudaError_t launch_ray(const ModelDev& m, const DataDev& d, const float* pnt, const float* vec, int nray, int pnt_nbatch, const int* geomgroup, int flg_static,
                       const int* bodyexclude, float* dist, int* geomid, float* normal, cudaStream_t s);
cudaError_t launch_ctrl_noise(const ModelDev& m, const DataDev& d, const float* ctrl_center, int step, float std, float rate, cudaStream_t s);
size_t smem_position(const ModelDev& m, const DataDev& d);
size_t smem_collision(const ModelDev& m, const DataDev& d);
size_t smem_constraint(const ModelDev& m, const DataDev& d);
size_t smem_velocity(const ModelDev& m, const DataDev& d, const FluidDev& f);
cudaError_t resident_worlds_position(const ModelDev& m, const DataDev& d, int* worlds);
cudaError_t resident_worlds_velocity(const ModelDev& m, const DataDev& d, int* worlds, const FluidDev& f);
size_t smem_solver(const ModelDev& m, const DataDev& d);
cudaError_t launch_set_const_fixed(const ModelDev& m, int nw, int nworld, cudaStream_t s);
cudaError_t launch_set_const_qpos(const ModelDev& m, const DataDev& d, const SetConstDev& c, int mode, int nw, cudaStream_t s);
cudaError_t launch_set_const_0(const ModelDev& m, const DataDev& d, const SetConstDev& c, int nw, cudaStream_t s);
cudaError_t launch_set_const_spring(const ModelDev& m, const DataDev& d, int nw, cudaStream_t s);
size_t smem_set_const(const ModelDev& m);
size_t smem_integrate(const ModelDev& m);
```

Baseline: 20.57 million.

## Pack tree/joint/dof index records and stage actuator inputs in shared memory

Adds packed int4 records per tree level slot, joint and dof, so the kinematics, com, crb and velocity tree passes read one vectorized cached load instead of several scattered index arrays. The velocity kernel also stages actuator moment structure, ctrl, lengths, qpos and qfrc_applied into shared memory asynchronously, overlapping with the backward force pass, and moves the actuator velocity computation to use the staged data. It also adds optional phase-clock instrumentation that is compiled out by default. This raises shared memory layout complexity and limits indices to 16 bits.

```diff
diff --git a/mujoco_warp_b200/_src/io.py b/mujoco_warp_b200/_src/io.py
--- a/mujoco_warp_b200/_src/io.py
+++ b/mujoco_warp_b200/_src/io.py
@@ -89,6 +89,30 @@
   return np.asarray(getattr(mjm, name))
 
 
+def tree_records(mjm, level_body, childadr) -> dict:
+  nbody = mjm.nbody
+  parent, jntadr, jntnum = _np(mjm, "body_parentid"), _np(mjm, "body_jntadr"), _np(mjm, "body_jntnum")
+  dofadr, dofnum = _np(mjm, "body_dofadr"), _np(mjm, "body_dofnum")
+  jtype, jqpos, jdof, jbody = _np(mjm, "jnt_type"), _np(mjm, "jnt_qposadr"), _np(mjm, "jnt_dofadr"), _np(mjm, "jnt_bodyid")
+  dbody, djnt = _np(mjm, "dof_bodyid"), _np(mjm, "dof_jntid")
+  childnum = np.diff(childadr)
+  if max(nbody, mjm.njnt, mjm.nv, int(childadr[-1])) >= 1 << 16 or (nbody and max(int(jntnum.max()), int(dofnum.max())) >= 1 << 8):
+    raise NotImplementedError("the packed tree records hold 16-bit body / joint / dof indices and at most 255 joints or dofs per body")
+  slot = np.zeros((nbody, 4), dtype=np.int64)
+  for i, b in enumerate(level_body):
+    nj, nd = int(jntnum[b]), int(dofnum[b])
+    slot[i, 0] = b | max(int(parent[b]), 0) << 16
+    slot[i, 1] = (int(jntadr[b]) | nj << 16 | int(jtype[jntadr[b]]) << 24) if nj else 0
+    slot[i, 2] = (int(dofadr[b]) | nd << 16) if nd else 0
+    slot[i, 3] = int(childadr[b]) | int(childnum[b]) << 16
+  jrec = np.stack([jtype, jqpos, jdof, jbody], axis=1) if mjm.njnt else np.zeros((1, 4))
+  drec = np.zeros((max(mjm.nv, 1), 4), dtype=np.int64)
+  for d in range(mjm.nv):
+    j = int(djnt[d])
+    drec[d] = (int(dbody[d]), j, int(jqpos[j]), int(jtype[j]) | (d - int(jdof[j])) << 8)
+  return {"level_slot": slot.astype(np.int32), "jnt_rec": np.asarray(jrec, dtype=np.int32), "dof_rec": drec.astype(np.int32)}
+
+
 def derive_tables(mjm) -> dict:
   nbody, nv, ngeom, njnt, nu = mjm.nbody, mjm.nv, mjm.ngeom, mjm.njnt, mjm.nu
   parent = _np(mjm, "body_parentid")
@@ -107,6 +131,7 @@
     children[parent[b]].append(b)
   t["body_childadr"] = np.concatenate([[0], np.cumsum([len(c) for c in children])]).astype(np.int32)
   t["body_childid"] = np.array([c for cs in children for c in cs] + ([0] if nbody == 1 else []), dtype=np.int32)
+  t.update(tree_records(mjm, order, t["body_childadr"]))
   rownnz, rowadr, colind = _np(mjm, "M_rownnz"), _np(mjm, "M_rowadr"), _np(mjm, "M_colind")
   nC = int(rownnz.sum())
   entry_row = np.zeros(nC, dtype=np.int32)
@@ -449,7 +474,7 @@
   m.ntenfric = int((np.asarray(mjm.tendon_frictionloss) > 0).sum()) if nt else 0
   m.jnt_limited = dev_i(np.asarray(mjm.jnt_limited).astype(np.int32))
   m.body_tree = tuple(dev_i(x) for x in t["body_tree"])
-  for n in ("body_childadr", "body_childid", "level_adr", "level_body", "M_entry_row", "mulm_rowadr", "mulm_col", "mulm_madr", "tree_qLDadr",
+  for n in ("body_childadr", "body_childid", "level_adr", "level_body", "level_slot", "jnt_rec", "dof_rec", "M_entry_row", "mulm_rowadr", "mulm_col", "mulm_madr", "tree_qLDadr",
             "qLD_block_adr", "jnt_limited_slide_hinge_adr", "jnt_limited_ball_adr", "dof_fricloss_adr", "moment_rownnz0", "moment_rowadr0", "moment_colind0",
             "dofact_adr", "dofact_act", "dofact_mom",
             "nxn_geom_pair", "nxn_pairid", "nxn_geom_pair_filtered", "nxn_pairid_filtered"):
@@ -564,7 +589,7 @@
     "jnt_limited_adr": m.jnt_limited_slide_hinge_adr, "nxn_geom_pair": m.nxn_geom_pair_filtered, "nxn_pairid": m.nxn_pairid_filtered,
     "body_isdofancestor": m._isdofancestor_nv, "meaninertia": m.stat.meaninertia,
   }
-  for n in (_FLOAT_FIELDS + _INT_FIELDS + ["body_childadr", "body_childid", "level_adr", "level_body", "M_entry_row", "mulm_rowadr", "mulm_col",
+  for n in (_FLOAT_FIELDS + _INT_FIELDS + ["body_childadr", "body_childid", "level_adr", "level_body", "level_slot", "jnt_rec", "dof_rec", "M_entry_row", "mulm_rowadr", "mulm_col",
                                          "mulm_madr", "tree_qLDadr", "dof_fricloss_adr", "moment_rownnz0", "moment_rowadr0", "moment_colind0",
                                          "dofact_adr", "dofact_act", "dofact_mom", "eq_type", "eq_obj1id", "eq_obj2id", "eq_solref", "eq_solimp", "eq_data",
                                          "jnt_limited_ball_adr", "pair_dim", "pair_friction", "pair_solref", "pair_solreffriction", "pair_solimp",
diff --git a/mujoco_warp_b200/csrc/k_position.cu b/mujoco_warp_b200/csrc/k_position.cu
--- a/mujoco_warp_b200/csrc/k_position.cu
+++ b/mujoco_warp_b200/csrc/k_position.cu
@@ -2,6 +2,9 @@
 #include "mjb_math.cuh"
 #include "mjb_team.cuh"
 #include "mjb_types.cuh"
+
+[[maybe_unused]] constexpr int POS_NCLK = 10;
+MJB_PHASE_CLOCK_BUFFER(pos_clk, mjb_phase_clocks_position)
 
 namespace {
 
@@ -42,6 +45,7 @@
   float* S = smem + (size_t)(threadIdx.x >> 5) * ((size_t)L.total * G + 4);
   Stager st;
   st.init(reinterpret_cast<uint64_t*>(S + (size_t)L.total * G), lane);
+  PHASE_CLOCK(pos_clk, POS_NCLK, 0);
   const int nb = m.nbody, nj = m.njnt, ng = m.ngeom, nv = m.nv;
 #define BLK(f) (S + (size_t)L.f * G)
 #define ROW(blk, n) ((blk) + (size_t)g * (n))
@@ -64,6 +68,7 @@
   }
   if (!com && (cam || crbm)) { GLOAD(BLK(scom), subtree_com, 3 * nb); GLOAD(BLK(cinert), cinert, 10 * nb); GLOAD(BLK(cdof), cdof, 6 * nv); }
   st.load_wait();
+  PHASE_CLOCK(pos_clk, POS_NCLK, 1);
 
   if (kin) {
     if (sub == 0) { xpos[0] = xpos[1] = xpos[2] = 0.f; xquat[0] = 1.f; xquat[1] = xquat[2] = xquat[3] = 0.f; }
@@ -72,9 +77,10 @@
     for (int l = 1; l < m.nlevel; l++) {
 #pragma unroll 1
       for (int i = m.level_adr[l] + sub; i < m.level_adr[l + 1]; i += LPW) {
-        const int b = m.level_body[i], pid = m.body_parentid[b], jntadr = m.body_jntadr[b], jntnum = m.body_jntnum[b];
-        if (jntnum == 1 && m.jnt_type[jntadr] == JNT_FREE) {
-          const int qa = m.jnt_qposadr[jntadr];
+        const TreeSlot ts = tree_slot(m, i);
+        const int b = ts.b, pid = ts.pid, jntadr = ts.jntadr, jntnum = ts.jntnum;
+        if (jntnum == 1 && ts.jtype0 == JNT_FREE) {
+          const int qa = jnt_rec(m, jntadr).y;
           v3 p = ld3(qpos + qa);
           q4 q = qnormalize(ldq(qpos + qa + 3));
           st3(xpos + 3 * b, p); stq(xquat + 4 * b, q);
@@ -89,7 +95,8 @@
         q4 quat = qmul(pq, bquat);
 #pragma unroll 1
         for (int j = jntadr; j < jntadr + jntnum; j++) {
-          const int qa = m.jnt_qposadr[j], t = m.jnt_type[j];
+          const int4 jr = jnt_rec(m, j);
+          const int qa = jr.y, t = jr.x;
           v3 jpos = ld3(m.jnt_pos + 3 * j), jax = ld3(m.jnt_axis + 3 * j);
           v3 anchor = qrot(quat, jpos) + pos, axis = qrot(quat, jax);
           if (t == JNT_BALL) {
@@ -108,6 +115,7 @@
       __syncwarp();
     }
   }
+  PHASE_CLOCK(pos_clk, POS_NCLK, 2);
 
   if (kin && m.ntendon > 0) {
 #pragma unroll 1
@@ -146,6 +154,7 @@
   }
 
   __syncwarp();
+  PHASE_CLOCK(pos_clk, POS_NCLK, 3);
 
   if (kin) {
 #pragma unroll 2
@@ -177,6 +186,7 @@
     }
   }
   __syncwarp();
+  PHASE_CLOCK(pos_clk, POS_NCLK, 4);
 
   if (com) {
 #pragma unroll 2
@@ -186,9 +196,10 @@
     for (int l = m.nlevel - 2; l >= 0; l--) {
 #pragma unroll 1
       for (int i = m.level_adr[l] + sub; i < m.level_adr[l + 1]; i += LPW) {
-        const int b = m.level_body[i];
+        const TreeSlot ts = tree_slot(m, i);
+        const int b = ts.b;
         v3 acc = ld3(scom + 3 * b);
-        for (int c = m.body_childadr[b]; c < m.body_childadr[b + 1]; c++) acc = acc + ld3(scom + 3 * m.body_childid[c]);
+        for (int c = ts.childadr; c < ts.childadr + ts.childnum; c++) acc = acc + ld3(scom + 3 * m.body_childid[c]);
         st3(scom + 3 * b, acc);
       }
       __syncwarp();
@@ -199,6 +210,7 @@
       if (ms != 0.f) st3(scom + 3 * b, ld3(scom + 3 * b) * (1.0f / ms));
     }
     __syncwarp();
+    PHASE_CLOCK(pos_clk, POS_NCLK, 5);
     if (kin) st.store_wait_read();
 #pragma unroll 2
     for (int b = sub; b < nb; b += LPW) {
@@ -221,8 +233,9 @@
     }
 #pragma unroll 2
     for (int j = sub; j < nj; j += LPW) {
-      const int b = m.jnt_bodyid[j], t = m.jnt_type[j];
-      int dof = m.jnt_dofadr[j];
+      const int4 jr = jnt_rec(m, j);
+      const int b = jr.w, t = jr.x;
+      int dof = jr.z;
       const v3 offset = ld3(scom + 3 * m.body_rootid[b]) - ld3(xanchor + 3 * j);
       if (t == JNT_FREE || t == JNT_BALL) {
         float xm[9];
@@ -249,6 +262,7 @@
     st.store_commit();
   }
   __syncwarp();
+  PHASE_CLOCK(pos_clk, POS_NCLK, 6);
 
   if (mask & STG_CAMLIGHT) {
 #pragma unroll 1
@@ -321,6 +335,7 @@
     GSTORE(geom_xpos, BLK(gxpos), 3 * ng); GSTORE(geom_xmat, BLK(gxmat), 9 * ng);
     st.store_commit();
   }
+  PHASE_CLOCK(pos_clk, POS_NCLK, 7);
 
   if (crbm) {
     st.store_wait_read();
@@ -328,12 +343,13 @@
     for (int l = m.nlevel - 2; l >= 1; l--) {
 #pragma unroll 1
       for (int i = m.level_adr[l] + sub; i < m.level_adr[l + 1]; i += LPW) {
-        const int b = m.level_body[i];
+        const TreeSlot ts = tree_slot(m, i);
+        const int b = ts.b;
         float acc[10];
 #pragma unroll
         for (int k = 0; k < 10; k++) acc[k] = crb[10 * b + k];
 #pragma unroll 1
-        for (int c = m.body_childadr[b]; c < m.body_childadr[b + 1]; c++) {
+        for (int c = ts.childadr; c < ts.childadr + ts.childnum; c++) {
           const float* cc = crb + 10 * m.body_childid[c];
 #pragma unroll
           for (int k = 0; k < 10; k++) acc[k] += cc[k];
@@ -343,6 +359,7 @@
       }
       __syncwarp();
     }
+    PHASE_CLOCK(pos_clk, POS_NCLK, 8);
 #pragma unroll 2
     for (int dd = sub; dd < nv; dd += LPW) inert_vec(crb + 10 * m.dof_bodyid[dd], cdof + 6 * dd, buf + 6 * dd);
     __syncwarp();
@@ -358,6 +375,7 @@
     st.store_commit();
   }
   st.store_wait_read();
+  PHASE_CLOCK(pos_clk, POS_NCLK, 9);
 #undef GLOAD
 #undef GSTORE
 #undef BLK
diff --git a/mujoco_warp_b200/csrc/k_velocity.cu b/mujoco_warp_b200/csrc/k_velocity.cu
--- a/mujoco_warp_b200/csrc/k_velocity.cu
+++ b/mujoco_warp_b200/csrc/k_velocity.cu
@@ -4,9 +4,12 @@
 #include "mjb_team.cuh"
 #include "mjb_types.cuh"
 
+[[maybe_unused]] constexpr int VEL_NCLK = 11;
+MJB_PHASE_CLOCK_BUFFER(vel_clk, mjb_phase_clocks_velocity)
+
 namespace {
 
-struct VelLayout { int qvel, cdof, cinert, cvel, cdofdot, cacc, cfrc, qpas, qbias, qact, qsm, qld, x, af, total; };
+struct VelLayout { int qvel, cdof, cinert, cvel, cdofdot, cacc, cfrc, qpas, qbias, qact, qsm, qld, x, af, avel, qpos, ctrl, alen, qapp, mnnz, madr, mcol, mmom, total; };
 __host__ __device__ inline VelLayout vel_layout(const ModelDev& m) {
   VelLayout L;
   int o = 0;
@@ -20,6 +23,13 @@
   L.cfrc = L.cdofdot;
   if (pad(m.nv) + pad(m.nu) <= L.cvel - L.cinert) { L.qact = L.cinert; L.af = L.cinert + pad(m.nv); }
   else { L.qact = take(m.nv); L.af = take(m.nu); }
+  auto place = [&](int& lo, int hi, int n) { if (lo + pad(n) <= hi) { const int r = lo; lo += pad(n); return r; } return take(n); };
+  int lo = L.qact == L.cinert ? L.af + pad(m.nu) : L.cinert;
+  L.mnnz = place(lo, L.qvel, m.nu); L.madr = place(lo, L.qvel, m.nu); L.mcol = place(lo, L.qvel, m.nJmom); L.mmom = place(lo, L.qvel, m.nJmom);
+  lo = L.cvel;
+  L.ctrl = place(lo, L.cdofdot, m.nu); L.alen = place(lo, L.cdofdot, m.nu); L.qapp = place(lo, L.cdofdot, m.nv); L.avel = place(lo, L.cdofdot, m.nu);
+  lo = L.cacc;
+  L.qpos = place(lo, L.cacc + pad(6 * m.nbody), m.nq);
   L.qld = a0;
   if (o - a0 < pad(m.qld_total)) o = a0 + pad(m.qld_total);
   L.total = o;
diff --git a/mujoco_warp_b200/csrc/k_velocity_body.cuh b/mujoco_warp_b200/csrc/k_velocity_body.cuh
--- a/mujoco_warp_b200/csrc/k_velocity_body.cuh
+++ b/mujoco_warp_b200/csrc/k_velocity_body.cuh
@@ -10,21 +10,29 @@
   float* S = smem + (size_t)(threadIdx.x >> 5) * ((size_t)L.total * G + 4);
   Stager st;
   st.init(reinterpret_cast<uint64_t*>(S + (size_t)L.total * G), lane);
+  PHASE_CLOCK(vel_clk, VEL_NCLK, 0);
   const int nv = m.nv, nb = m.nbody, nu = m.nu;
 #define FLD(f, n) (S + (size_t)L.f * G + (size_t)g * (n))
   float *qvel = FLD(qvel, nv), *cdof = FLD(cdof, 6 * nv), *cinert = FLD(cinert, 10 * nb), *cvel = FLD(cvel, 6 * nb), *cdofdot = FLD(cdofdot, 6 * nv),
         *cacc = FLD(cacc, 6 * nb), *cfrc = FLD(cfrc, 6 * nb), *q_passive = FLD(qpas, nv), *q_bias = FLD(qbias, nv), *q_act = FLD(qact, nv),
-        *q_smooth = FLD(qsm, nv), *qld = FLD(qld, m.qld_total), *x = FLD(x, nv), *aforce = FLD(af, nu);
+        *q_smooth = FLD(qsm, nv), *qld = FLD(qld, m.qld_total), *x = FLD(x, nv), *aforce = FLD(af, nu), *avel = FLD(avel, nu),
+        *sqpos = FLD(qpos, m.nq), *sctrl = FLD(ctrl, nu), *salen = FLD(alen, nu), *sqapp = FLD(qapp, nv), *smom = FLD(mmom, m.nJmom);
+  const int *smnnz = reinterpret_cast<const int*>(FLD(mnnz, nu)), *smadr = reinterpret_cast<const int*>(FLD(madr, nu)),
+            *smcol = reinterpret_cast<const int*>(FLD(mcol, m.nJmom));
   const float* Mw = d.M + (size_t)T.w * m.nC;
 #undef FLD
   const size_t wg = (size_t)T.wg0;
 #define GLOAD(f, field, n) st.load(S + (size_t)L.f * G, d.field + wg * (size_t)(n), nval * (n))
+#define GLOADI(f, field, n) st.load(S + (size_t)L.f * G, reinterpret_cast<const float*>(d.field + wg * (size_t)(n)), nval * (n))
 #define GSTORE(field, f, n) st.store(d.field + wg * (size_t)(n), S + (size_t)L.f * G, nval * (n))
   const size_t wb = (size_t)T.w;
   const bool v_all = mask & STG_VELOCITY;
+  bool staged = false;
 
   GLOAD(qvel, qvel, nv); GLOAD(cdof, cdof, 6 * nv);
   if (v_all || (mask & STG_RNE)) GLOAD(cinert, cinert, 10 * nb);
+  if (!FLUID && (v_all || (mask & STG_PASSIVE)) && !(m.disableflags & DSBL_SPRING)) GLOAD(qpos, qpos, m.nq);
+  const float* qsp = FLUID ? d.qpos + wb * m.nq : sqpos;
   constexpr int MREG = 32;
   float mreg[MREG];
   const bool fac = mask & (STG_ACCELERATION | STG_FACTOR_ONLY);
@@ -32,20 +40,13 @@
   for (int k = 0; k < MREG; k++) { const int e = sub + k * LPW; mreg[k] = (fac && e < m.nC) ? Mw[e] : 0.f; }
   bool any_xfrc = false;
   if (mask & STG_ACCELERATION) {
-#pragma unroll 4
+#pragma unroll 8
     for (int i = sub; i < 6 * nb; i += LPW) any_xfrc |= d.xfrc_applied[wb * 6 * nb + i] != 0.f;
   }
   st.load_wait();
+  PHASE_CLOCK(vel_clk, VEL_NCLK, 1);
 
   if (mask & (STG_VELOCITY | STG_COMVEL | STG_PASSIVE | STG_RNE)) {
-    if (v_all)
-#pragma unroll 1
-    for (int a = valid ? sub : nu; a < nu; a += LPW) {
-      const int nnz = d.moment_rownnz[wb * nu + a], adr = d.moment_rowadr[wb * nu + a];
-      float vel = 0.f;
-      for (int k = 0; k < nnz; k++) vel += d.actuator_moment[wb * m.nJmom + adr + k] * qvel[d.moment_colind[wb * m.nJmom + adr + k]];
-      d.actuator_velocity[wb * nu + a] = vel;
-    }
     if (PEXT && v_all && m.ntendon > 0) {
 #pragma unroll 1
       for (int t = valid ? sub : m.ntendon; t < m.ntendon; t += LPW) {
@@ -54,6 +55,7 @@
         d.ten_velocity[wb * m.ntendon + t] = vel;
       }
     }
+    PHASE_CLOCK(vel_clk, VEL_NCLK, 2);
     if (v_all || (mask & STG_COMVEL)) {
     if (sub < 6) cvel[sub] = 0.f;
     __syncwarp();
@@ -61,14 +63,16 @@
     for (int l = 1; l < m.nlevel; l++) {
 #pragma unroll 1
       for (int i = m.level_adr[l] + sub; i < m.level_adr[l + 1]; i += LPW) {
-        const int b = m.level_body[i], pid = m.body_parentid[b], jntadr = m.body_jntadr[b], jntnum = m.body_jntnum[b];
-        int dof = m.body_dofadr[b];
+        const TreeSlot ts = tree_slot(m, i);
+        const int b = ts.b, pid = ts.pid, jntadr = ts.jntadr, jntnum = ts.jntnum;
+        const bool one_dof = ts.dofnum == jntnum;
+        int dof = ts.dofadr;
         float cv[6];
 #pragma unroll
         for (int k = 0; k < 6; k++) cv[k] = cvel[6 * pid + k];
 #pragma unroll 1
         for (int j = jntadr; j < jntadr + jntnum; j++) {
-          const int t = m.jnt_type[j];
+          const int t = one_dof ? JNT_HINGE : j == jntadr ? ts.jtype0 : m.jnt_type[j];
           if (t == JNT_FREE) {
             for (int q = 0; q < 3; q++) { const float v = qvel[dof + q]; for (int k = 0; k < 6; k++) { cv[k] += cdof[6 * (dof + q) + k] * v; cdofdot[6 * (dof + q) + k] = 0.f; } }
             for (int q = 3; q < 6; q++) motion_cross(cv, cdof + 6 * (dof + q), cdofdot + 6 * (dof + q));
@@ -98,6 +102,7 @@
       st.load_wait();
     }
 
+    PHASE_CLOCK(vel_clk, VEL_NCLK, 3);
     if (v_all || (mask & STG_PASSIVE)) {
       const bool dsbl_spring = m.disableflags & DSBL_SPRING, dsbl_damper = m.disableflags & DSBL_DAMPER;
       const bool gravcomp = PEXT && m.has_gravcomp && !(m.disableflags & DSBL_GRAVITY) && !(dsbl_spring && dsbl_damper);
@@ -113,18 +118,19 @@
       }
 #pragma unroll 1
       for (int dd = sub; dd < nv; dd += LPW) {
-        const int j = m.dof_jntid[dd], t = m.jnt_type[j];
+        const int4 dr = dof_rec(m, dd);
+        const int j = dr.y, t = dr.w & 0xff;
         float spring = 0.f, damper = 0.f, gc = 0.f;
         if (!(dsbl_spring && dsbl_damper)) {
           const float stiffness = m.jnt_stiffness[j];
           if (stiffness != 0.f && !dsbl_spring) {
-            const int qa = m.jnt_qposadr[j], k = dd - m.jnt_dofadr[j];
-            if (t == JNT_SLIDE || t == JNT_HINGE) spring = -(d.qpos[wb * m.nq + qa] - m.qpos_spring[qa]) * stiffness;
+            const int qa = dr.z, k = dr.w >> 8;
+            if (t == JNT_SLIDE || t == JNT_HINGE) spring = -(qsp[qa] - m.qpos_spring[qa]) * stiffness;
             else if (!PEXT) {}
-            else if (t == JNT_FREE && k < 3) spring = -stiffness * (d.qpos[wb * m.nq + qa + k] - m.qpos_spring[qa + k]);
+            else if (t == JNT_FREE && k < 3) spring = -stiffness * (qsp[qa + k] - m.qpos_spring[qa + k]);
             else {
               const int ra = t == JNT_FREE ? qa + 3 : qa, kk = t == JNT_FREE ? k - 3 : k;
-              const q4 rot = qnormalize(ldq(d.qpos + wb * m.nq + ra)), ref = ldq(m.qpos_spring + ra);
+              const q4 rot = qnormalize(ldq(qsp + ra)), ref = ldq(m.qpos_spring + ra);
               const q4 qd = qmul(mkq(ref.w, -ref.x, -ref.y, -ref.z), rot);
               const float s2 = sqrtf(qd.x * qd.x + qd.y * qd.y + qd.z * qd.z);
               if (s2 != 0.f) {
@@ -182,20 +188,23 @@
         }
       }
     }
+    PHASE_CLOCK(vel_clk, VEL_NCLK, 4);
     if (v_all || (mask & STG_RNE)) {
+    __syncwarp();
     for (int k = sub; k < 6; k += LPW) cacc[k] = k < 3 ? 0.f : ((m.disableflags & DSBL_GRAVITY) ? 0.f : -(k == 3 ? m.gravity_x : k == 4 ? m.gravity_y : m.gravity_z));
     __syncwarp();
 #pragma unroll 1
     for (int l = 1; l < m.nlevel; l++) {
 #pragma unroll 1
       for (int i = m.level_adr[l] + sub; i < m.level_adr[l + 1]; i += LPW) {
-        const int b = m.level_body[i], pid = m.body_parentid[b];
+        const TreeSlot ts = tree_slot(m, i);
+        const int b = ts.b, pid = ts.pid;
         float a[6];
 #pragma unroll
         for (int k = 0; k < 6; k++) a[k] = cacc[6 * pid + k];
 #pragma unroll 1
-        for (int q = 0; q < m.body_dofnum[b]; q++) {
-          const int dof = m.body_dofadr[b] + q;
+        for (int q = 0; q < ts.dofnum; q++) {
+          const int dof = ts.dofadr + q;
           const float v = qvel[dof];
 #pragma unroll
           for (int k = 0; k < 6; k++) a[k] += cdofdot[6 * dof + k] * v;
@@ -205,6 +214,7 @@
       }
       __syncwarp();
     }
+    PHASE_CLOCK(vel_clk, VEL_NCLK, 5);
     st.store_wait_read();
 #pragma unroll 2
     for (int b = sub; b < nb; b += LPW) {
@@ -221,16 +231,23 @@
       for (int k = 0; k < 6; k++) cfrc[6 * b + k] = f[k];
     }
     __syncwarp();
+    if (v_all) {
+      GLOADI(mnnz, moment_rownnz, nu); GLOADI(madr, moment_rowadr, nu); GLOADI(mcol, moment_colind, m.nJmom); GLOAD(mmom, actuator_moment, m.nJmom);
+      if (mask & STG_ACTUATION) { GLOAD(ctrl, ctrl, nu); GLOAD(alen, actuator_length, nu); }
+      if (mask & STG_ACCELERATION) GLOAD(qapp, qfrc_applied, nv);
+      staged = true;
+    }
 #pragma unroll 1
     for (int l = m.nlevel - 2; l >= 0; l--) {
 #pragma unroll 1
       for (int i = m.level_adr[l] + sub; i < m.level_adr[l + 1]; i += LPW) {
-        const int b = m.level_body[i];
+        const TreeSlot ts = tree_slot(m, i);
+        const int b = ts.b;
         float acc[6];
 #pragma unroll
         for (int k = 0; k < 6; k++) acc[k] = cfrc[6 * b + k];
 #pragma unroll 1
-        for (int c = m.body_childadr[b]; c < m.body_childadr[b + 1]; c++) {
+        for (int c = ts.childadr; c < ts.childadr + ts.childnum; c++) {
           const float* cc = cfrc + 6 * m.body_childid[c];
 #pragma unroll
           for (int k = 0; k < 6; k++) acc[k] += cc[k];
@@ -248,12 +265,31 @@
     st.store_fence();
     GSTORE(cacc, cacc, 6 * nb); GSTORE(cfrc_int, cfrc, 6 * nb); GSTORE(qfrc_bias, qbias, nv);
     st.store_commit();
+    PHASE_CLOCK(vel_clk, VEL_NCLK, 6);
     }
   } else if (mask & STG_ACCELERATION) {
     GLOAD(qpas, qfrc_passive, nv); GLOAD(qbias, qfrc_bias, nv);
     st.load_wait();
   }
-  __syncwarp();
+  if (!staged) {
+    st.store_wait_read();
+    if (mask & STG_ACTUATION) {
+      GLOAD(ctrl, ctrl, nu); GLOAD(alen, actuator_length, nu); GLOAD(avel, actuator_velocity, nu); GLOAD(mmom, actuator_moment, m.nJmom);
+    }
+    if (mask & STG_ACCELERATION) GLOAD(qapp, qfrc_applied, nv);
+  }
+  st.load_wait();
+  if (v_all) {
+#pragma unroll 1
+    for (int a = valid ? sub : nu; a < nu; a += LPW) {
+      const int nnz = smnnz[a], adr = smadr[a];
+      float vel = 0.f;
+      for (int k = 0; k < nnz; k++) vel += smom[adr + k] * qvel[smcol[adr + k]];
+      d.actuator_velocity[wb * nu + a] = vel;
+      avel[a] = vel;
+    }
+    __syncwarp();
+  }
 
   if (mask & STG_ACTUATION) {
 #pragma unroll 1
@@ -264,9 +300,9 @@
     for (int a = sub; a < nu; a += LPW) {
       float force = 0.f;
       if (enabled) {
-        float ctrl = d.ctrl[wb * nu + a];
+        float ctrl = sctrl[a];
         if (m.actuator_ctrllimited[a] && !(m.disableflags & DSBL_CLAMPCTRL)) ctrl = clampf(ctrl, m.actuator_ctrlrange[2 * a], m.actuator_ctrlrange[2 * a + 1]);
-        const float length = d.actuator_length[wb * nu + a], velocity = d.actuator_velocity[wb * nu + a];
+        const float length = salen[a], velocity = avel[a];
         const float *gp = m.actuator_gainprm + 10 * a, *bp = m.actuator_biasprm + 10 * a;
         float gain = 0.f, bias = 0.f;
         if (m.actuator_gaintype[a] == GAIN_FIXED) gain = gp[0];
@@ -309,7 +345,7 @@
 #pragma unroll 1
       for (int dd = sub; dd < nv; dd += LPW) {
         float q = 0.f;
-        for (int k = m.dofact_adr[dd]; k < m.dofact_adr[dd + 1]; k++) q += d.actuator_moment[wb * m.nJmom + m.dofact_mom[k]] * aforce[m.dofact_act[k]];
+        for (int k = m.dofact_adr[dd]; k < m.dofact_adr[dd + 1]; k++) q += smom[m.dofact_mom[k]] * aforce[m.dofact_act[k]];
         const int j = m.dof_jntid[dd];
         if (!(m.disableflags & DSBL_GRAVITY) && m.jnt_actgravcomp[j]) q += d.qfrc_gravcomp[wb * nv + dd];
         if (m.jnt_actfrclimited[j]) q = clampf(q, m.jnt_actfrcrange[2 * j], m.jnt_actfrcrange[2 * j + 1]);
@@ -324,11 +360,12 @@
     st.load_wait();
   }
   __syncwarp();
+  PHASE_CLOCK(vel_clk, VEL_NCLK, 7);
 
   if (mask & (STG_ACCELERATION | STG_FACTOR_ONLY)) {
     if (mask & STG_ACCELERATION) {
 #pragma unroll 1
-      for (int dd = sub; dd < nv; dd += LPW) q_smooth[dd] = q_passive[dd] - q_bias[dd] + q_act[dd] + d.qfrc_applied[wb * nv + dd];
+      for (int dd = sub; dd < nv; dd += LPW) q_smooth[dd] = q_passive[dd] - q_bias[dd] + q_act[dd] + sqapp[dd];
       if (team_any<LPW>(any_xfrc, g)) {
 #pragma unroll 1
         for (int dd = sub; dd < nv; dd += LPW) {
@@ -358,6 +395,7 @@
 #pragma unroll 1
       for (int i = sub; i < nv; i += LPW) x[i] = q_smooth[i];
     __syncwarp();
+    PHASE_CLOCK(vel_clk, VEL_NCLK, 8);
 #pragma unroll 1
     for (int t = 0; t < m.ntree; t++) {
       const int start = m.tree_dofadr[t], n = m.tree_dofnum[t];
@@ -372,6 +410,7 @@
       for (int e = max(e0, MREG * LPW) + ((sub - max(e0, MREG * LPW)) % LPW + LPW) % LPW; e < e1; e += LPW)
         U[(m.M_colind[e] - start) * n + (m.M_entry_row[e] - start)] = Mw[e];
       __syncwarp();
+      PHASE_CLOCK(vel_clk, VEL_NCLK, 9);
       team_chol_upper<LPW>(U, n, x + start, acc, sub);
     }
     st.store_fence();
@@ -380,5 +419,7 @@
     st.store_commit();
   }
   st.store_wait_read();
+  PHASE_CLOCK(vel_clk, VEL_NCLK, 10);
 #undef GLOAD
+#undef GLOADI
 #undef GSTORE
diff --git a/mujoco_warp_b200/csrc/mjb_team.cuh b/mujoco_warp_b200/csrc/mjb_team.cuh
--- a/mujoco_warp_b200/csrc/mjb_team.cuh
+++ b/mujoco_warp_b200/csrc/mjb_team.cuh
@@ -92,6 +92,30 @@
   }
 };
 
+struct TreeSlot { int b, pid, jntadr, jntnum, jtype0, dofadr, dofnum, childadr, childnum; };
+__device__ __forceinline__ TreeSlot tree_slot(const ModelDev& m, int i) {
+  const int4 r = __ldg(reinterpret_cast<const int4*>(m.level_slot) + i);
+  TreeSlot s;
+  s.b = r.x & 0xffff; s.pid = (int)((unsigned)r.x >> 16);
+  s.jntadr = r.y & 0xffff; s.jntnum = (r.y >> 16) & 0xff; s.jtype0 = (int)((unsigned)r.y >> 24);
+  s.dofadr = r.z & 0xffff; s.dofnum = (int)((unsigned)r.z >> 16);
+  s.childadr = r.w & 0xffff; s.childnum = (int)((unsigned)r.w >> 16);
+  return s;
+}
+__device__ __forceinline__ int4 jnt_rec(const ModelDev& m, int j) { return __ldg(reinterpret_cast<const int4*>(m.jnt_rec) + j); }
+__device__ __forceinline__ int4 dof_rec(const ModelDev& m, int d) { return __ldg(reinterpret_cast<const int4*>(m.dof_rec) + d); }
+
+#ifdef MJB_PHASE_CLOCKS
+#define MJB_PHASE_CLOCK_BUFFER(buf, setter)                          \
+  __device__ unsigned long long* buf;                                \
+  extern "C" int setter(void* p) { return (int)cudaMemcpyToSymbol(buf, &p, sizeof(p)); }
+#define PHASE_CLOCK(buf, n, k) \
+  do { if (lane == 0 && buf) buf[(size_t)(T.wg0 / G) * (n) + (k)] = clock64(); } while (0)
+#else
+#define MJB_PHASE_CLOCK_BUFFER(buf, setter)
+#define PHASE_CLOCK(buf, n, k) do {} while (0)
+#endif
+
 using TeamKernel = void (*)(ModelDev, DataDev, int);
 template <class K>
 using TeamChooserOf = K (*)(const ModelDev& m, int lpw);
diff --git a/mujoco_warp_b200/csrc/mjb_types.cuh b/mujoco_warp_b200/csrc/mjb_types.cuh
--- a/mujoco_warp_b200/csrc/mjb_types.cuh
+++ b/mujoco_warp_b200/csrc/mjb_types.cuh
@@ -9,7 +9,7 @@
   X(timestep) X(tolerance) X(ls_tolerance) X(impratio_invsqrt) X(meaninertia) X(gravity_x) X(gravity_y) X(gravity_z) X(ccd_tolerance)
 #define MJB_MODEL_IARRS(X) \
   X(body_parentid) X(body_rootid) X(body_weldid) X(body_mocapid) X(body_jntnum) X(body_jntadr) X(body_dofnum) X(body_dofadr) \
-  X(body_childadr) X(body_childid) X(level_adr) X(level_body) \
+  X(body_childadr) X(body_childid) X(level_adr) X(level_body) X(level_slot) X(jnt_rec) X(dof_rec) \
   X(jnt_type) X(jnt_qposadr) X(jnt_dofadr) X(jnt_bodyid) X(jnt_actfrclimited) X(jnt_actgravcomp) X(jnt_limited_adr) \
   X(dof_bodyid) X(dof_jntid) X(dof_parentid) X(dof_fricloss_adr) X(M_rownnz) X(M_rowadr) X(M_colind) X(M_entry_row) X(mulm_rowadr) X(mulm_col) X(mulm_madr) \
   X(tree_dofadr) X(tree_dofnum) X(tree_qLDadr) \
```

After: 20.91 million (median of 6 runs). 1.02x the previous value.
